# RomanJuranek/librectify

Measured on AMD Instinct MI355X. Metric: Mpix/s end-to-end (detect+VP) on 4K frames, batch call of 64 frames, 5 in flight, higher is better.
Workload: dtype f32

## Files before the change

### librectify_amd/csrc/batch.hip

```cpp
#include "host.h"

#include <cstdio>
#include <cstdlib>
#include <cstring>
#include <string>

namespace lramd {


class LaneSet {
public:
    LaneSet() = default;
    LaneSet(const LaneSet&) = delete;
    LaneSet& operator=(const LaneSet&) = delete;
    int setup(lr_context* caller, int S, bool host_frames, bool keep_workspace) {
        c = caller;
        c->workers.reserve((size_t)std::max(0, S - 1));
        while ((int)c->workers.size() < S - 1) {
            lr_context* wc = nullptr;
            if (ctx_create(c->device, &wc)) return 1;
            c->workers.push_back(wc);
        }
        lanes.reserve((size_t)S);
        lanes.push_back(c);
        for (int i = 0; i < S - 1; ++i) lanes.push_back(c->workers[i]);
        for (lr_context* l : lanes) {
            l->opt = c->opt;
            l->flood_log_min = S == 1 ? 0 : 32;
            l->flood_log_walk = S == 1 ? 0 : 24;
            l->flood_logbig_off = S > 1;
            l->flood_jit_sleep_us = S == 1 ? 0 : 20;
            static const bool sleep_env = std::getenv("LIBRECTIFY_LANES_SLEEP") != nullptr;
            l->sleep_in_wait = sleep_env && host_frames;
            l->keep_workspace = keep_workspace;
        }
        return 0;
    }
    ~LaneSet() {
        if (!c) return;
        for (lr_context* l : lanes) {
            l->sleep_in_wait = false;
            l->keep_workspace = false;
        }
        c->flood_logbig_off = false;
        c->flood_log_min = c->flood_log_walk = 0;
        c->flood_jit_sleep_us = 0;
    }
    int size() const { return (int)lanes.size(); }
    lr_context* operator[](int i) const { return lanes[(size_t)i]; }

private:
    lr_context* c = nullptr;
    std::vector<lr_context*> lanes;
};

struct BatchOut {
    LineSegment* out;
    int capacity;
    int* n_lines;
    const RectificationConfig* cfg;
    ImageTransform* transforms;
    void write(int b, const std::vector<LineSegment>& res, int w, int h) const {
        const int n = (int)res.size();
        if (n_lines) n_lines[b] = n;
        if (out && capacity > 0 && n > 0) std::memcpy(out + (size_t)b * capacity, res.data(), sizeof(LineSegment) * (size_t)std::min(n, capacity));
        if (transforms) {
            const RectificationConfig def;
            transforms[b] = rectification_transform(res.data(), std::min(n, capacity > 0 ? capacity : n), w, h, cfg ? *cfg : def);
        }
    }
};

template <class Frame>
static int run_lanes(const LaneSet& lanes, int batch, std::atomic<int>& stop, const Frame& frame) {
    const int S = lanes.size();
    std::atomic<int> next_frame{0};
    std::vector<int> rc((size_t)S, 0);
    std::vector<std::string> err((size_t)S);
    auto work = [&](int si) {
        bool failed = false;
        if (si > 0 && hipSetDevice(lanes[0]->device) != hipSuccess) {
            set_error("hipSetDevice failed");
            failed = true;
        }
        while (!failed && !stop.load(std::memory_order_relaxed)) {
            const int b = next_frame.fetch_add(1, std::memory_order_relaxed);
            if (b >= batch) break;
            failed = frame(lanes[si], si, b) != 0;
        }
        if (failed) {
            rc[(size_t)si] = 1;
            err[(size_t)si] = get_error();
            stop.store(1);
        }
    };
    {
        JoinedThreads workers;
        for (int si = 1; si < S; ++si) workers.th.emplace_back(work, si);
        work(0);
    }
    for (int si = 0; si < S; ++si)
        if (rc[(size_t)si]) {
            set_error(err[(size_t)si]);
            return 1;
        }
    return 0;
}

int ctx_find_groups_batch_device(lr_context* c, const void* d_images, int format, size_t image_stride, int batch, int w, int h,
                                 int stride, float min_length, bool refine, LineSegment* out, int capacity, int* n_lines,
                                 const RectificationConfig* cfg, ImageTransform* transforms) {
    if (batch <= 0) return 0;
    const size_t bpp = (size_t)pix_bytes(format);
    if (bpp == 0) {
        set_error("unknown pixel format of the frames");
        return 1;
    }
    LaneSet lanes;
    if (lanes.setup(c, std::max(1, std::min(c->opt.batch_streams, batch)), false, false)) return 1;
    const BatchOut results{out, capacity, n_lines, cfg, transforms};
    std::atomic<int> stop{0};
    return run_lanes(lanes, batch, stop, [&](lr_context* l, int, int b) {
        std::vector<LineSegment> res;
        if (ctx_find_groups_device(l, static_cast<const uint8_t*>(d_images) + (size_t)b * image_stride * bpp, format, w, h, stride, min_length,
                                   refine, res))
            return 1;
        results.write(b, res, w, h);
        return 0;
    });
}

int ctx_find_groups_frames_device(lr_context* c, const lr_frame* frames, int format, bool tagged, int batch, float min_length,
                                  bool refine, LineSegment* out, int capacity, int* n_lines, const RectificationConfig* cfg,
                                  ImageTransform* transforms) {
    auto bad = [](int b, const char* what) {
        set_error("lr_find_line_segment_groups_batch_device: frame " + std::to_string(b) + " of the table: " + what);
        return 1;
    };
    if (pix_bytes(format) == 0) {
        set_error("unknown pixel format of the frames");
        return 1;
    }
    if (frames == nullptr) {
        set_error("lr_find_line_segment_groups_batch_device: no frame table");
        return 1;
    }
    size_t max_pix = 0;
    int max_tiles = 0;
    for (int b = 0; b < batch; ++b) {
        const lr_frame& f = frames[b];
        if (f.data == nullptr) return bad(b, "null data");
        if (f.width < 1 || f.height < 1) return bad(b, "size below 1");
        if (f.stride < f.width) return bad(b, "stride smaller than the width");
        if (format == LR_PIX_F32 && (reinterpret_cast<uintptr_t>(f.data) & 3u)) return bad(b, "f32 address not 4-byte aligned");
        if (f.width < 5 || f.height < 5) {
            if (!tagged) return bad(b, "image smaller than the 5x5 filter");
            continue;
        }
        max_pix = std::max(max_pix, (size_t)f.width * (size_t)f.height);
        max_tiles = std::max(max_tiles, filter_geometry(f.width, f.height).n_tiles);
    }
    LaneSet lanes;
    if (lanes.setup(c, std::max(1, std::min(c->opt.batch_streams, batch)), false, true)) return 1;
    LR_HIP(hipSetDevice(c->device));
    for (int si = 0; si < lanes.size() && max_pix; ++si)
        if (ctx_reserve_workspace(lanes[si], max_pix, max_tiles)) return 1;
    const BatchOut results{out, capacity, n_lines, cfg, transforms};
    std::atomic<int> stop{0};
    return run_lanes(lanes, batch, stop, [&](lr_context* l, int, int b) {
        const lr_frame& f = frames[b];
        std::vector<LineSegment> res;
        if (f.width >= 5 && f.height >= 5 &&
            ctx_find_groups_device(l, f.data, format, f.width, f.height, f.stride, f.min_length < 0.f ? min_length : f.min_length, refine, res))
            return 1;
        results.write(b, res, f.width, f.height);
        return 0;
    });
}

int ctx_find_groups_batch_host(lr_context* c, const void* const* frames, int format, int batch, int w, int h, int stride,
                               float min_length, bool refine, int num_threads, LineSegment* out, int capacity,
                               int* n_lines, const RectificationConfig* cfg, ImageTransform* transforms) {
    if (batch <= 0) return 0;
    const int bpp = pix_bytes(format);
    if (bpp == 0) {
        set_error("unknown pixel format of the frames");
        return 1;
    }
    const int S = std::max(1, std::min(c->opt.batch_streams, batch));
    BatchUploader up(c, frames, batch, w, h, stride, bpp, S, num_threads);
    if (up.check()) return 1;
    LaneSet lanes;
    if (lanes.setup(c, S, true, false) || up.start()) return 1;
    const BatchOut results{out, capacity, n_lines, cfg, transforms};
    const int lanes_rc = run_lanes(lanes, batch, up.stop, [&](lr_context* l, int si, int b) {
        const void* img = nullptr;
        int slot = -1;
        if (up.ready(b, l->stream, &img, &slot)) return 1;
        if (img == nullptr) return 0;
        std::vector<LineSegment> res;
        const double t_f0 = now_ms();
        if (ctx_find_groups_device(l, img, format, w, h, w, min_length, refine, res)) return 1;
        up.release(slot, b, l, si, t_f0);
        results.write(b, res, w, h);
        return 0;
    });
    const std::string& up_err = up.end();
    if (lanes_rc) return 1;
    if (!up_err.empty()) {
        set_error(up_err);
        return 1;
    }
    return 0;
}

int ctx_find_groups_batch_host_multi(lr_context* c, const int* devices, int n_devices, const void* const* frames, int format, int batch,
                                     int w, int h, int stride, float min_length, bool refine, int num_threads,
                                     LineSegment* out, int capacity, int* n_lines, const RectificationConfig* cfg,
                                     ImageTransform* transforms) {
    if (batch <= 0) return 0;
    if (n_devices <= 0 || devices == nullptr) {
        set_error("multi-device batch: empty device list");
        return 1;
    }
    int ndev = 0;
    if (hipGetDeviceCount(&ndev) != hipSuccess) ndev = 0;
    for (int i = 0; i < n_devices; ++i)
        if (devices[i] < 0 || devices[i] >= ndev) {
            set_error("multi-device batch: device index out of range");
            return 1;
        }
    if ((int)c->peers.size() > n_devices) {
        for (size_t i = (size_t)n_devices; i < c->peers.size(); ++i) ctx_destroy(c->peers[i]);
        c->peers.resize((size_t)n_devices);
    }
    c->peers.resize((size_t)n_devices, nullptr);
    for (int i = 0; i < n_devices; ++i) {
        if (c->peers[(size_t)i] && c->peers[(size_t)i]->device != devices[i]) {
            ctx_destroy(c->peers[(size_t)i]);
            c->peers[(size_t)i] = nullptr;
        }
        if (!c->peers[(size_t)i] && ctx_create(devices[i], &c->peers[(size_t)i])) {
            (void)hipSetDevice(c->device);
            return 1;
        }
        c->peers[(size_t)i]->opt = c->opt;
    }
    const int per = (batch + n_devices - 1) / n_devices;
    bool blocks_apart = true;
    if (const size_t fbpp = (size_t)pix_bytes(format)) {
        const size_t span = (size_t)(h - 1) * (size_t)(stride < 0 ? -stride : stride) * fbpp + (size_t)w * fbpp;
        for (int i = 0; i < batch && blocks_apart && w > 0 && h > 0; ++i)
            for (int j = (i / per + 1) * per; j < batch && blocks_apart; ++j) {
                if (!frames[i] || !frames[j]) continue;
                const uintptr_t a = reinterpret_cast<uintptr_t>(frames[i]) - (stride < 0 ? (size_t)(h - 1) * (size_t)(-stride) * fbpp : 0);
                const uintptr_t b = reinterpret_cast<uintptr_t>(frames[j]) - (stride < 0 ? (size_t)(h - 1) * (size_t)(-stride) * fbpp : 0);
                blocks_apart = a + span <= b || b + span <= a;
            }
    }
    for (lr_context* p : c->peers) p->batch_no_register = !blocks_apart;
    std::vector<int> rc((size_t)n_devices, 0);
    std::vector<std::string> err((size_t)n_devices);
    auto run = [&](int i) {
        const int b0 = std::min(batch, i * per), b1 = std::min(batch, b0 + per);
        if (b1 <= b0) return;
        lr_context* p = c->peers[(size_t)i];
        if (hipSetDevice(p->device) != hipSuccess) {
            rc[(size_t)i] = 1;
            err[(size_t)i] = "hipSetDevice failed";
            return;
        }
        const int nt = num_threads > 1 ? std::max(2, num_threads / std::min(n_devices, (batch + per - 1) / per)) : num_threads;
        if (ctx_find_groups_batch_host(p, frames + b0, format, b1 - b0, w, h, stride, min_length, refine, nt,
                                       out ? out + (size_t)b0 * capacity : nullptr, capacity, n_lines ? n_lines + b0 : nullptr, cfg,
                                       transforms ? transforms + b0 : nullptr)) {
            rc[(size_t)i] = 1;
            err[(size_t)i] = get_error();
        }
    };
    std::vector<std::thread> th;
    for (int i = 1; i < n_devices; ++i) th.emplace_back(run, i);
    run(0);
    for (auto& t : th) t.join();
    (void)hipSetDevice(c->device);
    for (int i = 0; i < n_devices; ++i)
        if (rc[(size_t)i]) {
            set_error("device list entry " + std::to_string(i) + " (device " + std::to_string(devices[i]) + "): " + err[(size_t)i]);
// ... 7 lines not shown
```

### librectify_amd/csrc/common.h

```cpp
#pragma once
#include <hip/hip_runtime.h>

#include <cstdint>
#include <string>

#include "../../include/librectify_amd.h"

namespace lramd {

constexpr float kEps = 1e-6f;
constexpr int kMaxModels = 4;
constexpr int kMaxPeelModels = 5;
constexpr float kInlierDeg = 2.0f;
constexpr float kGarbageDeg = 4.0f;
constexpr int kRansacMaxIter = 10000;
constexpr int kEdgeKernelSize = 2;
constexpr float kEdgeKernelSigma = 1.0f;
constexpr int kSeedDist = 2;
constexpr float kSeedRatio = 0.95f;
constexpr float kTraceTolerance = 0.25f;
constexpr float kLineMaxErr = 2.0f;
constexpr float kLineMinLength = 5.f;
constexpr int kComponentMinSize = 5;
constexpr int kBins = 8;
constexpr int kOverlayStrokeNum = 9, kOverlayStrokeDen = 4;
constexpr int kOverlayDiscR2 = 25;
constexpr int kOverlayColours = 12;
constexpr uint32_t kOverlayPalette[kOverlayColours] = {0x0000FFu, 0x00FF00u, 0xFF0000u, 0xFFFF00u, 0xFF00FFu, 0x00FFFFu,
                                                       0x000080u, 0x008000u, 0x800000u, 0x808000u, 0x800080u, 0x008080u};
constexpr uint32_t kOverlayUngrouped = 0xFFFFFFu;
constexpr int kOverlayMaxCoord = 1 << 24;

struct FilterConsts {
    float d[5];
    float g[5];
    float st[kBins];
    float ct[kBins];
};

struct BinTrig {
    float st[kBins];
    float ct[kBins];
};

constexpr uint32_t kLabelFree = 0xFFFFFFFFu;

__host__ __device__ inline float directional(float dx, float dy, float s, float c) {
    return fabsf(fmaf(dx, s, dy * c));
}

__host__ __device__ inline uint64_t splitmix64(uint64_t x) {
    x += 0x9E3779B97F4A7C15ull;
    x = (x ^ (x >> 30)) * 0xBF58476D1CE4E5B9ull;
    x = (x ^ (x >> 27)) * 0x94D049BB133111EBull;
    return x ^ (x >> 31);
}
__host__ __device__ inline void sample_pair(uint64_t seed, uint32_t round, uint32_t iter, uint32_t n, uint32_t& a,
                                            uint32_t& b) {
    const uint64_t z = splitmix64(seed ^ splitmix64(((uint64_t)round << 32) | iter));
    const uint32_t u1 = (uint32_t)z, u2 = (uint32_t)(z >> 32);
    const uint32_t i = (uint32_t)(((uint64_t)u1 * n) >> 32);
    uint32_t j = (uint32_t)(((uint64_t)u2 * (n - 1)) >> 32);
    if (j >= i) ++j;
    a = i < j ? i : j;
    b = i < j ? j : i;
}

void set_error(const std::string& msg);

#define LR_HIP(expr)                                                                                     \
    do {                                                                                                 \
        hipError_t _e = (expr);                                                                          \
        if (_e != hipSuccess) {                                                                          \
            (void)hipGetLastError();        \
            ::lramd::set_error(std::string(#expr) + ": " + hipGetErrorString(_e) + " (" + __FILE__ + ":" + \
                               std::to_string(__LINE__) + ")");                                          \
            return 1;                                                                                    \
        }                                                                                                \
    } while (0)

inline int pix_bytes(int format) { return format == LR_PIX_U8 ? 1 : format == LR_PIX_U8X3 ? 3 : format == LR_PIX_F32 ? 4 : 0; }
int launch_filter(const void* img, int format, int w, int h, int stride, const FilterConsts& fc, float* dx, float* dy,
                  uint8_t* dmask, uint64_t* cand, uint32_t* cand_count, uint32_t* tile_max, hipStream_t s);
int filter_band_rows();
int filter_band_last_row(int by);
int launch_filter_rows(const void* img, int format, int w, int h, int stride, const FilterConsts& fc, float* dx, float* dy,
                       uint8_t* dmask, uint64_t* cand, uint32_t* cand_count, uint32_t* tile_max, int by_begin, int by_end,
                       hipStream_t s);
struct FilterGeom {
    int n_tiles;
    int cand_cap;
};
FilterGeom filter_geometry(int w, int h);

size_t seeds_temp_bytes(int n_tiles, size_t max_seeds);
int launch_seed_select(const uint64_t* cand, const uint32_t* cand_count, const uint32_t* tile_max, int n_tiles,
                       int cand_cap, float seed_keep_ratio, float* maxmag, uint32_t* tile_pass, uint32_t* tile_off, uint64_t* keys,
                       uint32_t key_cap, uint32_t* n_seeds, uint32_t frame_tag, hipStream_t s);
int launch_seed_order(uint64_t* keys, uint64_t* keys_alt, const uint32_t* n_seeds, uint32_t cap, const float* dx, const float* dy,
                      BinTrig trig, float trace_tolerance, int32_t* seed_idx, int32_t* seed_bin, float* seed_thr, uint4* seed_rec, hipStream_t s);

int launch_label_init(uint32_t* label, size_t n, hipStream_t s);
int launch_flood_ordered(const float* dx, const float* dy, const uint8_t* dmask, int w, int h, const int32_t* seed_idx,
                         const int32_t* seed_bin, const float* seed_thr, const uint32_t* d_n_seeds, uint32_t seed_cap,
                         BinTrig trig, uint32_t* label, int32_t* seed_size, int32_t* queue, hipStream_t s);

constexpr size_t kFloodHandWords = 1024;
struct FloodBuffers {
    uint32_t* blocked = nullptr;
    uint32_t* count = nullptr;
    uint32_t* flags = nullptr;
    uint8_t* state = nullptr;
    uint8_t* tier = nullptr;
    uint32_t* blk = nullptr;
    uint32_t* act_a = nullptr;
    uint32_t* act_b = nullptr;
    uint32_t* ctrl = nullptr;
    uint8_t* dirty = nullptr;
    uint32_t* big_list = nullptr;
    uint32_t* handover = nullptr;
    bool rewalk_logs = false;
    uint32_t* rewalk_list = nullptr;
    int log_min_tiles = 0, log_walk_tiles = 0;
    bool giant_hold = false;
    bool giant_step = true;
    void* giant_mask = nullptr;
    uint32_t* giant_parent = nullptr;
    bool log_sweep = false;
    bool rewalk_big = false;
    uint32_t log_seeds = 0, log_cap = 0;
    uint32_t* log_off = nullptr;
    uint32_t* log_len = nullptr;
    uint32_t* log_buf = nullptr;
    void* slab_ring = nullptr;
    void* slab_hash = nullptr;
    uint32_t n_slabs = 0, slab_ring_cap = 0, slab_hash_cap = 0;
    int win_first_shift = 0, win_growth = 2;
    int win_hold_pct = 80;
    bool partial_commits = true;
    bool second_tier = true;
    bool second_tier_from_start = true;
    bool hold_from_start = false;
    bool staged_from_start = false;
    int blind_rounds = 10;
    uint32_t* host_progress = nullptr;
    bool calm_hint = false;
    uint32_t* host_ctrl = nullptr;
    int jit_first = 0;
    int jit_sleep_us = 0;
// ... 116 lines not shown
```

### librectify_amd/csrc/context.h

```cpp
#pragma once
#include <atomic>
#include <functional>
#include <memory>
#include <mutex>
#include <vector>

#include "buffers.h"
#include "common.h"
#include "vp_host.h"

namespace lramd {
struct StagingCrew;

struct Settings {
    uint64_t ransac_seed = 0;
    int ransac_iters = kRansacMaxIter;
    int estimator = 0;
    int prosac_T_N = -1;
    int cht_d = 128;
    int batch_streams = 5;
    int flood_mode = 1;
    bool flood_giant_step = true;
    bool flood_jit = true;
    bool flood_partial = true;
// ... 29 lines not shown
    HugeSort huge;
};

struct FloodStore {
    DeviceBuffer<uint32_t> blocked, count, flags, blk, act_a, act_b, ctrl, big_list, handover, rewalk_list, log_off, log_len, log_buf;
    DeviceBuffer<uint8_t> state, tier, dirty;
    DeviceBuffer<uint64_t> giant_mask;
    DeviceBuffer<uint4> slab_ring, slab_hash;
    FloodBuffers fb;
    size_t cap_seeds = 0;
};

struct FrameSlots {
    DeviceBuffer<float> slot[2];
    PinnedBuffer<float> stage[2];
    DeviceBuffer<float> packed;
    DeviceBuffer<float> luma;
};

struct UploadRing {
    std::vector<DeviceBuffer<float>> img;
    std::vector<PinnedBuffer<float>> stage;
    size_t cap_pix = 0, stage_cap_pix = 0;
    void drop() {
        for (auto& b : img) b.reset();
        for (auto& b : stage) b.reset();
        cap_pix = stage_cap_pix = 0;
    }
};

struct PrepareSpans {
    MirroredBuffer<unsigned char> spans;
    int key[4] = {0, 0, 0, 0};
    float w_in[2] = {0.f, 0.f};
    MirroredBuffer<unsigned char> ragged;
};

struct OverlayStore {
    MirroredBuffer<unsigned char> block;
};

struct JpegStore {
    MirroredBuffer<unsigned char> block;
    DeviceBuffer<int16_t> coef;
    DeviceBuffer<uint32_t> len;
    DeviceBuffer<unsigned long long> place;
    DeviceBuffer<unsigned long long> counts;
};

struct JpegDecodeStore {
    MirroredBuffer<unsigned char> block;
    DeviceBuffer<int16_t> coef;
    DeviceBuffer<unsigned long long> state;
    DeviceBuffer<uint32_t> part;
};
}

struct lr_context {
    lr_context();
    ~lr_context();
    int device = 0;
    lramd::Stream stream, copy_stream;
    lramd::Settings opt;

    int w = 0, h = 0;
    lramd::Workspace ws;
    lramd::FloodStore flood;
    lramd::FrameSlots frames;
    lramd::UploadRing ring;
    lramd::PrepareSpans prep;
    lramd::Event ev_prep_spans;
    lramd::Event ev_prep_ragged;
    lramd::OverlayStore overlay;
    lramd::Event ev_overlay;
    lramd::JpegStore jpeg;

    lramd::Event ev_up[2];
    lramd::Event ev_wait;
    std::vector<lramd::Event> band_ev;
    std::vector<lramd::Event> ring_ev;
    std::unique_ptr<lramd::StagingCrew> crew;
    int crew_helpers = 0;
    bool sleep_in_wait = false;
    uint32_t fit_tag = 0;
    bool batch_no_register = false;
    int register_slow_calls = 0;
    uint32_t select_tag = 0;
    lramd::DeviceBuffer<float> maxmag;
    lramd::DeviceBuffer<uint32_t> d_counts;
    uint32_t seed_cap = 0;
    uint32_t seed_cap_once = 0;
    int frame_laps = 0;
    lramd::FloodProgress flood_prog;
    bool keep_workspace = false;
    int small_frames = 0;
    size_t cap_glines = 0;
    lramd::DeviceBuffer<float> d_tables;
    lramd::DeviceBuffer<uint32_t> d_orig;
    lramd::DeviceBuffer<float> d_inl;
    lramd::DeviceBuffer<LineSegment> d_flines;
    lramd::DeviceBuffer<uint32_t> d_gctl;
    lramd::DeviceBuffer<float> d_gnorm;
    lramd::DeviceBuffer<float> d_models;
    lramd::PinnedBuffer<uint8_t> h_res;
    size_t res_lines_cap = 0;
    lramd::DeviceBuffer<float> d_refine_table;
    lramd::DeviceBuffer<uint2> d_refine_edges;
    lramd::DeviceBuffer<unsigned long long> d_cht_acc;
    lramd::MirroredBuffer<uint32_t> cht_idx;
    lramd::MirroredBuffer<uint32_t> cht_peak;
    lramd::MirroredBuffer<double> warp_m;
    lramd::Event ev_warp_m;
    lramd::MirroredBuffer<float> model;
    lramd::DeviceBuffer<unsigned long long> d_best_slots;
    lramd::MirroredBuffer<int32_t> pairs;
    lramd::DeviceBuffer<float> d_peak;
    lramd::MirroredBuffer<float> weights;
    lramd::MirroredBuffer<uint32_t> samples;
    lramd::MirroredBuffer<uint32_t> hcounts;
    lramd::MirroredBuffer<uint32_t> rec;
    lramd::MirroredBuffer<uint8_t> recflags;
    lramd::Event prosac_ev[2];
    std::vector<int> prosac_imin;
    std::vector<lr_context*> workers;
    std::vector<lr_context*> peers;
    lramd::PinnedBuffer<uint32_t> h_counts;
    lramd::PinnedBuffer<float> h_best;

    lramd::FilterConsts fconsts;
    lramd::BinTrig trig;
    float seed_keep_ratio = 0.f;

    uint32_t n_seeds = 0, n_comp = 0, n_px = 0;
    int flood_rounds = 0;
    int flood_rounds_hint = 10;
    int flood_rounds_last = 0;
    int flood_jit_sleep_us = 0;
    bool flood_logbig_off = false;
    int flood_log_min = 0, flood_log_walk = 0;
    bool flood_logbig_hint = true;
    bool flood_big_hint = true;
    bool flood_hold_hint = false;
    int flood_staged_streak = 0;
    bool flood_staged_hint = false;
    bool flood_calm_hint = false;
    uint32_t flood_tiers[16] = {0, 0, 0, 0, 0, 0, 0, 0, 0, 0, 0, 0, 0, 0, 0, 0};
    lramd::Event ev[16];
    float stage_ms[LR_T_COUNT] = {};
    double host_ms[3] = {0, 0, 0};
    bool stage_valid[4] = {false, false, false, false};
    bool dmask_consumed = false;
    lramd::JpegDecodeStore jpeg_decode;
};

namespace lramd {
constexpr size_t kResHeaderBytes = 256;
int ctx_create(int device, lr_context** out);
void ctx_destroy(lr_context* c);
const std::string& get_error();
int ctx_ensure_image_capacity(lr_context* c, int w, int h);
int ctx_reserve_workspace(lr_context* c, size_t npix, int ntiles);
int ctx_trim(lr_context* c, bool frames_too);
int ctx_ensure_ransac_capacity(lr_context* c, size_t n_lines);
int ctx_stage_filter(lr_context* c, const float* d_image, int w, int h, int stride);
int ctx_stage_seeds(lr_context* c);
int ctx_stage_flood(lr_context* c);
// ... 74 lines not shown
```

### librectify_amd/csrc/frame.hip

```cpp
#include "host.h"

#include <cstdio>
#include <cstdlib>
#include <cstring>

namespace lramd {


namespace {

uint32_t round_up(uint32_t v, uint32_t m) { return (v + m - 1) / m * m; }

uint32_t initial_seed_cap(size_t npix) {
    return (uint32_t)std::min<size_t>(npix, std::max<size_t>(round_up((uint32_t)(npix / 32), 1024), 4096));
}

uint32_t line_cap_for(const lr_context* c) {
    return (uint32_t)std::min<size_t>(c->seed_cap, c->ws.cap_pix / 6 + 16);
}


PencilTable table_of(lr_context* c, int which) {
    const size_t cl = c->cap_glines;
    float* b = c->d_tables + (size_t)which * 8 * cl;
// ... 307 lines not shown
    c->stage_valid[1] = true;
    return 0;
}

int ctx_stage_flood(lr_context* c) {
    if (!c->stage_valid[1]) {
        set_error(c->dmask_consumed ? "lr_stage_flood: the previous flood consumed the filter output; run lr_stage_filter and lr_stage_seeds again"
                                    : "lr_stage_flood: run lr_stage_seeds first");
        return 1;
    }
    TimingOn t(c);
    if (enqueue_flood(c)) return 1;
    LR_HIP(hipStreamSynchronize(c->stream));
    bool extra;
    if (finish_flood(c, &extra)) return 1;
    c->stage_valid[2] = true;
    return 0;
}

int ctx_stage_fit(lr_context* c, std::vector<LineSegment>& out) {
    if (!c->stage_valid[2]) {
        set_error("lr_stage_fit: run lr_stage_flood first");
        return 1;
    }
    out.clear();
    TimingOn t(c);
    if (enqueue_fit(c)) return 1;
    LR_HIP(hipMemcpyAsync(c->h_counts, c->d_counts, 8 * sizeof(uint32_t), hipMemcpyDeviceToHost, c->stream));
    LR_HIP(hipStreamSynchronize(c->stream));
    c->n_comp = c->h_counts[kCntComp];
    c->n_px = c->h_counts[kCntPx];
    if (c->n_comp > 0) {
        out.resize(c->n_comp);
        LR_HIP(hipMemcpyAsync(out.data(), c->ws.d_lines, (size_t)c->n_comp * sizeof(LineSegment), hipMemcpyDeviceToHost,
                              c->stream));
        LR_HIP(hipStreamSynchronize(c->stream));
    }
    c->stage_valid[3] = true;
    record_stage_times(c, false);
    return 0;
}

int ctx_detect(lr_context* c, const float* d_image, int w, int h, int stride, std::vector<LineSegment>& raw) {
    if (ctx_stage_filter(c, d_image, w, h, stride)) return 1;
    if (ctx_stage_seeds(c)) return 1;
    if (ctx_stage_flood(c)) return 1;
    return ctx_stage_fit(c, raw);
}

int run_frame(lr_context* c, const void* d_image, int format, int w, int h, int stride, float min_length, bool refine,
              std::vector<LineSegment>& out, bool filter_enqueued) {
    out.clear();
    const double t_begin = now_ms();
    const bool fused = !refine && c->opt.estimator == 0;
    const int n_iter = c->opt.ransac_iters;
    auto groups_after_fit = [&]() -> int {
        const uint32_t lc = line_cap_for(c);
        if (ensure_group_capacity(c, lc)) return 1;
        if (ensure_result_block(c, std::max<size_t>(c->res_lines_cap, 4096))) return 1;
        if (c->opt.timing_on) LR_HIP(hipEventRecord(c->ev[5], c->stream));
        const PencilTable all = table_of(c, 0), round0 = table_of(c, 1);
        if (launch_filter_lines(c->ws.d_lines, c->d_counts + kCntComp, lc, min_length, c->d_flines, c->d_gctl, c->d_gnorm, &all, &round0,
                                c->stream))
            return 1;
        static_assert(kMaxModels >= 1 && kGcWords == 8 && kResHeaderBytes == 256, "the last peeling round carries the result block (peel_kernel)");
        if (enqueue_groups(c, lc, kMaxModels, kInlierDeg, kGarbageDeg, n_iter, c->opt.ransac_seed, true, true)) return 1;
        if (c->opt.timing_on) LR_HIP(hipEventRecord(c->ev[6], c->stream));
        return 0;
    };
    auto after_fit = [&]() -> int {
        if (fused) return groups_after_fit();
        LR_HIP(hipMemcpyAsync(c->h_counts, c->d_counts, 8 * sizeof(uint32_t), hipMemcpyDeviceToHost, c->stream));
        return 0;
    };
    c->frame_laps = 0;
    for (int attempt = 0;; ++attempt) {
        c->frame_laps += 1;
        if (!(filter_enqueued && attempt == 0) && enqueue_filter(c, d_image, format, w, h, stride)) return 1;
        if (enqueue_seeds(c)) return 1;
        if (enqueue_flood(c)) return 1;
        if (enqueue_fit(c)) return 1;
        if (after_fit()) return 1;
        const double t_enq = now_ms();
        const double t_pre = now_ms();
        if (c->sleep_in_wait) {
            LR_HIP(hipEventRecord(c->ev_wait, c->stream));
            LR_HIP(hipEventSynchronize(c->ev_wait));
        } else {
            LR_HIP(hipStreamSynchronize(c->stream));
        }
        c->host_ms[0] = t_enq - t_begin;
        c->host_ms[1] = t_pre - t_enq;
        c->host_ms[2] = now_ms() - t_pre;
        const uint32_t* cnt = fused ? reinterpret_cast<const uint32_t*>(c->h_res.get()) : c->h_counts.get();
        c->n_seeds = cnt[kCntSeeds];
        if (c->n_seeds <= c->seed_cap) break;
        if (attempt > 0) {
            set_error("seed count exceeds the sort capacity twice");
            return 1;
        }
        adapt_seed_cap(c, c->n_seeds);
    }
    bool extra = false;
    if (finish_flood(c, &extra)) return 1;
    if (extra) {
        c->frame_laps += 1;
        if (enqueue_fit(c)) return 1;
        if (after_fit()) return 1;
        LR_HIP(hipStreamSynchronize(c->stream));
    }
    const uint32_t* cnt = fused ? reinterpret_cast<const uint32_t*>(c->h_res.get()) : c->h_counts.get();
    c->n_comp = cnt[kCntComp];
    c->n_px = cnt[kCntPx];
    adapt_seed_cap(c, c->n_seeds);
    c->stage_valid[0] = c->stage_valid[1] = false;
    c->stage_valid[2] = c->stage_valid[3] = true;
    if (fused) {
        const uint32_t* gctl = reinterpret_cast<const uint32_t*>(c->h_res + 32);
        const size_t n = gctl[kGcLines];
        out.resize(n);
        const size_t have = std::min<size_t>(n, c->res_lines_cap);
        if (have) std::memcpy(out.data(), c->h_res + kResHeaderBytes, have * sizeof(LineSegment));
        if (n > have) {
            LR_HIP(hipMemcpyAsync(out.data() + have, c->d_flines + have, (n - have) * sizeof(LineSegment),
                                  hipMemcpyDeviceToHost, c->stream));
            LR_HIP(hipStreamSynchronize(c->stream));
            if (ensure_result_block(c, round_up((uint32_t)(n + n / 2), 1024))) return 1;
        }
        record_stage_times(c, true);
#ifdef LR_PEEL_TIMING
        {
            const float* tm = reinterpret_cast<const float*>(c->h_res + 64) + 16;
            for (int r = 0; r < 4; ++r)
                std::fprintf(stderr, "peel round %d: best %.1f us, inliers %.1f, sums %.1f, jacobi %.1f, verdict %.1f\n", r,
                             tm[r * 5], tm[r * 5 + 1], tm[r * 5 + 2], tm[r * 5 + 3], tm[r * 5 + 4]);
        }
#endif
        return 0;
    }
    std::vector<LineSegment> raw(c->n_comp);
    if (c->n_comp) {
        LR_HIP(hipMemcpyAsync(raw.data(), c->ws.d_lines, (size_t)c->n_comp * sizeof(LineSegment), hipMemcpyDeviceToHost,
                              c->stream));
        LR_HIP(hipStreamSynchronize(c->stream));
    }
    record_stage_times(c, false);
    if (raw.size() < 2) return 0;
    if (refine && ctx_refine(c, raw)) return 1;
    std::vector<LineSegment> filtered = filter_lines(raw, min_length);
    if (filtered.empty()) return 0;
    if (c->opt.timing_on) LR_HIP(hipEventRecord(c->ev[5], c->stream));
    if (c->opt.estimator == 1) {
        if (ctx_estimate_line_pencils_prosac(c, filtered, kMaxModels, kInlierDeg, kGarbageDeg, c->opt.prosac_T_N,
                                             c->opt.ransac_seed))
            return 1;
    } else if (c->opt.estimator == 2) {
        if (ctx_estimate_line_pencils_direct(c, filtered, kMaxModels, kInlierDeg, kGarbageDeg)) return 1;
    } else if (c->opt.estimator == 3) {
        if (ctx_estimate_line_pencils_cht(c, filtered, kMaxModels, kInlierDeg, kGarbageDeg, c->opt.cht_d, nullptr)) return 1;
    } else if (ctx_estimate_line_pencils(c, filtered, kMaxModels, kInlierDeg, kGarbageDeg, n_iter, c->opt.ransac_seed)) {
        return 1;
    }
    if (c->opt.timing_on) LR_HIP(hipEventRecord(c->ev[6], c->stream));
    LR_HIP(hipStreamSynchronize(c->stream));
    record_stage_times(c, true);
    out.swap(filtered);
// ... 145 lines not shown
```

### librectify_amd/csrc/kernels_filter.hip

```cpp
#include <algorithm>
#include <cstdlib>
#include <cstring>

#include "common.h"

namespace lramd {
namespace {

struct FilterTaps {
    float d1, d2, g1, g2;
    float st[kBins];
    float ct[kBins];
};

#ifndef LR_BAND_ROWS
#define LR_BAND_ROWS 30
#endif
constexpr int kBandRows = LR_BAND_ROWS;
constexpr int kBandSteps = kBandRows + 8;

__device__ __forceinline__ float from_lower(float v) {
    const int i = __float_as_int(v);
    return __int_as_float(__builtin_amdgcn_mov_dpp(i, 0x138 , 0xF, 0xF, true));
}
// ... 66 lines not shown
template <int kFormat, int K10>
__device__ __forceinline__ void lane_step(Roll1<typename Px<kFormat>::Q>& R, const int t, const void* __restrict__ img, const int w, const int h,
                                          const int stride, const FilterTaps& fc, float* __restrict__ dx_out,
                                          float* __restrict__ dy_out, uint8_t* __restrict__ dmask_out,
                                          uint64_t* __restrict__ cand_band, uint32_t& ncand, float& lmax, const int y0,
                                          const int x, const int xcl, const int lane, const bool useful,
                                          const BufRsrc r_img, const BufRsrc r_dx, const BufRsrc r_dy,
                                          const BufRsrc r_dm) {
    constexpr int K = K10 % 5;
    if (t >= kBandSteps) return;
    const float cur = Px<kFormat>::value(R.q[K10]);
    {
        const int yy = min(max(y0 - 4 + t + 9, 0), h - 1);
        R.q[(K10 + 9) % 10] = Px<kFormat>::fetch(r_img, (unsigned)xcl, (unsigned)yy * (unsigned)stride);
    }
    const float l1 = from_lower(cur), r1 = from_upper(cur);
    const float l2 = from_lower(l1), r2 = from_upper(r1);
    R.hx[K] = fmaf(r2 - l2, fc.d2, (r1 - l1) * fc.d1);
    R.hs[K] = fmaf(r2 + l2, fc.g2, fmaf(r1 + l1, fc.g1, cur));
    if (t < 4) return;

    const int yc = y0 - 6 + t;
    const float ax = fmaf(R.hx[K] + R.hx[(K + 1) % 5], fc.g2,
                          fmaf(R.hx[(K + 4) % 5] + R.hx[(K + 2) % 5], fc.g1, R.hx[(K + 3) % 5]));
    const float ay = fmaf(R.hs[K] - R.hs[(K + 1) % 5], fc.d2, (R.hs[(K + 4) % 5] - R.hs[(K + 2) % 5]) * fc.d1);
    const bool ok = (yc >= 2) && (yc < h - 2) && (x >= 2) && (x < w - 2);
    const float vx = ok ? ax : 0.f;
    const float vy = ok ? ay : 0.f;
    R.mag[K] = sqrtf(vx * vx + vy * vy);
    float g[kBins];
#pragma unroll
    for (int b = 0; b < kBins; ++b) g[b] = directional(vx, vy, fc.st[b], fc.ct[b]);

    const float gm = fmaxf(fmaxf(fmaxf(g[0], g[1]), fmaxf(g[2], g[3])), fmaxf(fmaxf(g[4], g[5]), fmaxf(g[6], g[7])));
    uint32_t bit = 1u << 7;
#pragma unroll
    for (int b = kBins - 2; b >= 0; --b) bit = (g[b] == gm) ? (1u << b) : bit;
    R.bits[K] = bit;
    const bool in_img = useful && x < w;
    if (t >= 6 && t < 6 + kBandRows && yc < h) {
        if (in_img) {
            const unsigned row = (unsigned)yc * (unsigned)w * 4u;
            __builtin_amdgcn_raw_buffer_store_b32(__builtin_bit_cast(int, vx), r_dx, (unsigned)x * 4u, row, 0);
            __builtin_amdgcn_raw_buffer_store_b32(__builtin_bit_cast(int, vy), r_dy, (unsigned)x * 4u, row, 0);
        }
    }
    if (t < 8) return;

    const int yo = yc - 2;
    if (yo >= h) return;
    const float cm = fmaxf(fmaxf(fmaxf(R.mag[0], R.mag[1]), fmaxf(R.mag[2], R.mag[3])), R.mag[4]);
    const float cl1 = from_lower(cm), cr1 = from_upper(cm);
    const float cl2 = from_lower(cl1), cr2 = from_upper(cr1);
    const float mx = fmaxf(fmaxf(fmaxf(cl2, cl1), fmaxf(cm, cr1)), cr2);
    const float c = R.mag[(K + 3) % 5];
    const uint32_t cb = R.bits[(K + 3) % 5];
    const uint32_t v = R.bits[(K + 2) % 5] | cb | R.bits[(K + 4) % 5];
    uint32_t dm = from_lower(v) | v | from_upper(v);
    if (yo == 0 || yo == h - 1 || x == 0 || x == w - 1) dm = 0;
    if (in_img) {
        lmax = fmaxf(lmax, c);
        __builtin_amdgcn_raw_buffer_store_b8((unsigned char)dm, r_dm, (unsigned)x, (unsigned)yo * (unsigned)w, 0);
    }
    const bool peak = in_img && (yo >= 2) && (yo < h - 2) && (x >= 2) && (x < w - 2) && (c > 0.f) && (c == mx);
    const uint64_t m = __ballot(peak);
    if (m) {
        if (peak) {
            const uint32_t idx = (uint32_t)yo * (uint32_t)w + (uint32_t)x;
            const uint32_t pb = (uint32_t)__ffs((int)cb) - 1u;
            cand_band[ncand + (uint32_t)__popcll(m & ((1ull << lane) - 1ull))] =
                ((uint64_t)__float_as_uint(c) << 32) | (uint64_t)((idx << 3) | pb);
        }
        ncand += (uint32_t)__popcll(m);
    }
}

template <int kFormat>
__global__ __launch_bounds__(256) void filter_lanes_kernel(const void* __restrict__ img, int w, int h, int stride,
                                                           FilterTaps fc, float* __restrict__ dx_out,
                                                           float* __restrict__ dy_out, uint8_t* __restrict__ dmask_out,
                                                           uint64_t* __restrict__ cand, uint32_t* __restrict__ cand_count,
                                                           uint32_t* __restrict__ tile_max, int bands_x, int band_begin,
                                                           int band_end) {
    const int lane = threadIdx.x & 63;
#ifndef LR_NO_XCD_ORDER
    const int chunk = (int)gridDim.x / 8;
    const int wg = (int)(blockIdx.x & 7u) * chunk + (int)(blockIdx.x >> 3);
#else
    const int wg = (int)blockIdx.x;
#endif
    const int band = __builtin_amdgcn_readfirstlane(band_begin + wg * 4 + (int)(threadIdx.x >> 6));
    if (band >= band_end) return;
    const int by = band / bands_x, bx = band - by * bands_x;
    const int y0 = by * kBandRows;
    const int x = bx * kLaneCols - 4 + lane;
    const int xcl = min(max(x, 0), w - 1);
    const bool useful = lane >= 4 && lane <= 59;
    using P = Px<kFormat>;
    Roll1<typename P::Q> R;
#pragma unroll
    for (int i = 0; i < 5; ++i) {
        R.hx[i] = 0.f;
        R.hs[i] = 0.f;
        R.mag[i] = 0.f;
        R.bits[i] = 1u;
    }
#pragma unroll
    for (int i = 0; i < 10; ++i) R.q[i] = (i < 9) ? P::first(img, stride, h, y0 - 4 + i, xcl) : typename P::Q(0);
    uint64_t* cand_band = cand + (size_t)band * (kLaneCols * kBandRows);
    uint32_t ncand = 0;
    float lmax = 0.f;
    const uint32_t npx = (uint32_t)w * (uint32_t)h;
    const BufRsrc r_img = make_rsrc(img, ((uint32_t)(h - 1) * (uint32_t)stride + (uint32_t)w) * P::kBytes);
    const BufRsrc r_dx = make_rsrc(dx_out, npx * 4u), r_dy = make_rsrc(dy_out, npx * 4u), r_dm = make_rsrc(dmask_out, npx);
#define LR_STEP(k) lane_step<kFormat, k>(R, t0 + k, img, w, h, stride, fc, dx_out, dy_out, dmask_out, cand_band, ncand, lmax, y0, x, xcl, lane, useful, r_img, r_dx, r_dy, r_dm)
#pragma unroll
    for (int t0 = 0; t0 < (kBandSteps + 9) / 10 * 10; t0 += 10) {
        LR_STEP(0); LR_STEP(1); LR_STEP(2); LR_STEP(3); LR_STEP(4);
        LR_STEP(5); LR_STEP(6); LR_STEP(7); LR_STEP(8); LR_STEP(9);
    }
#undef LR_STEP
#pragma unroll
    for (int off = 32; off >= 1; off >>= 1) lmax = fmaxf(lmax, __shfl_xor(lmax, off));
    if (lane == 0) {
        tile_max[band] = __float_as_uint(lmax);
        cand_count[band] = ncand;
    }
}

}

FilterGeom filter_geometry(int w, int h) {
    FilterGeom g;
    g.n_tiles = ((w + kLaneCols - 1) / kLaneCols) * ((h + kBandRows - 1) / kBandRows);
    g.cand_cap = kLaneCols * kBandRows;
    return g;
}

static int filter_taps(const FilterConsts& fc, FilterTaps& ft) {
    if (!(fc.d[2] == 0.f && fc.g[2] == 1.f && fc.d[1] == -fc.d[3] && fc.d[0] == -fc.d[4] && fc.g[1] == fc.g[3] &&
          fc.g[0] == fc.g[4])) {
        set_error("launch_filter: derivative factors are not (anti)symmetric on this host");
        return 1;
    }
    ft.d1 = fc.d[3];
    ft.d2 = fc.d[4];
    ft.g1 = fc.g[3];
    ft.g2 = fc.g[4];
    for (int b = 0; b < kBins; ++b) {
        ft.st[b] = fc.st[b];
        ft.ct[b] = fc.ct[b];
    }
    return 0;
}

int filter_band_rows() { return kBandRows; }
int filter_band_last_row(int by) { return kBandRows * by - 4 + kBandSteps - 1; }

int launch_filter_rows(const void* img, int format, int w, int h, int stride, const FilterConsts& fc, float* dx, float* dy,
                       uint8_t* dmask, uint64_t* cand, uint32_t* cand_count, uint32_t* tile_max, int by_begin, int by_end,
                       hipStream_t s) {
    if (w < 1 || h < 1 || stride < w) {
        set_error("launch_filter: bad geometry");
        return 1;
    }
    if (format != LR_PIX_F32 && format != LR_PIX_U8) {
// ... 33 lines not shown
```

### librectify_amd/csrc/kernels_fit.hip

```cpp
#include <algorithm>
#include <cstring>

#include <atomic>

#include "common.h"

namespace lramd {
namespace {

constexpr uint32_t kNoComp = 0xFFFFFFFFu;

constexpr uint32_t kSortLds = 1024;
constexpr uint32_t kSortLdsBig = 16384;
constexpr uint32_t kHugeShift = 14;
constexpr uint32_t kHugeFlag = 0x80000000u;
constexpr int kOffPer = 8;
constexpr uint32_t kOffChunk = 256 * kOffPer;

__device__ __forceinline__ void chunk_counts(const int32_t* __restrict__ seed_size, uint32_t n_seeds, int min_size,
                                             uint32_t k0, int (&sz)[kOffPer], uint32_t& c, uint32_t& p) {
    c = p = 0;
#pragma unroll
    for (int j = 0; j < kOffPer; ++j) {
        sz[j] = (k0 + j < n_seeds) ? seed_size[k0 + j] : 0;
        if (sz[j] > min_size) {
            c += 1u;
            p += (uint32_t)sz[j];
        }
    }
}

__global__ __launch_bounds__(256) void component_offsets_kernel(const int32_t* __restrict__ seed_size,
                                                                const uint32_t* __restrict__ n_ptr, uint32_t cap,
                                                                int min_size, unsigned long long* __restrict__ status, uint32_t tag,
                                                                uint32_t* __restrict__ comp_rank,
                                                                uint32_t* __restrict__ comp_seed,
                                                                uint32_t* __restrict__ comp_off,
                                                                uint32_t* __restrict__ totals,
                                                                uint32_t* __restrict__ large_list,
                                                                uint32_t large_cap, uint32_t* __restrict__ n_large,
                                                                uint32_t* __restrict__ cursor, uint32_t* __restrict__ huge_list,
                                                                uint32_t huge_max) {
    __shared__ uint32_t s_c[4], s_p[4], s_cc[4], s_cp[4];
    const uint32_t n_seeds = min(*n_ptr, cap);
    const int tid = threadIdx.x, lane = tid & 63, wv = tid >> 6;
    const uint32_t k0 = blockIdx.x * kOffChunk + (uint32_t)tid * kOffPer;
    int sz[kOffPer];
    uint32_t c, p;
    chunk_counts(seed_size, n_seeds, min_size, k0, sz, c, p);
    uint32_t ic = c, ip = p;
#pragma unroll
    for (int off = 1; off < 64; off <<= 1) {
        const uint32_t tc = (uint32_t)__shfl_up((int)ic, off);
        const uint32_t tp = (uint32_t)__shfl_up((int)ip, off);
        if (lane >= off) {
            ic += tc;
            ip += tp;
        }
    }
    if (lane == 63) {
        s_c[wv] = ic;
        s_p[wv] = ip;
    }
    __syncthreads();
    if (tid == 0) {
        const unsigned long long t = (unsigned long long)tag << 32;
        const unsigned long long wc = t | (unsigned long long)(s_c[0] + s_c[1] + s_c[2] + s_c[3]);
        const unsigned long long wp = t | (unsigned long long)(s_p[0] + s_p[1] + s_p[2] + s_p[3]);
        if (blockIdx.x == 0) {
#pragma unroll
            for (int i = 0; i < 4; ++i) __hip_atomic_store(&n_large[i], 0u, __ATOMIC_RELAXED, __HIP_MEMORY_SCOPE_AGENT);
            __hip_atomic_store(&status[0], wc, __ATOMIC_RELEASE, __HIP_MEMORY_SCOPE_AGENT);
            __hip_atomic_store(&status[1], wp, __ATOMIC_RELEASE, __HIP_MEMORY_SCOPE_AGENT);
        } else {
            __hip_atomic_store(&status[2u * blockIdx.x], wc, __ATOMIC_RELAXED, __HIP_MEMORY_SCOPE_AGENT);
            __hip_atomic_store(&status[2u * blockIdx.x + 1u], wp, __ATOMIC_RELAXED, __HIP_MEMORY_SCOPE_AGENT);
        }
    }
    uint32_t cc = 0, cp = 0;
    for (uint32_t i = (uint32_t)tid; i < blockIdx.x; i += 256) {
        unsigned long long wc = 0ull, wp = 0ull;
        for (uint32_t spins = 0; spins < (1u << 22); ++spins) {
            wc = __hip_atomic_load(&status[2u * i], __ATOMIC_RELAXED, __HIP_MEMORY_SCOPE_AGENT);
            wp = __hip_atomic_load(&status[2u * i + 1u], __ATOMIC_RELAXED, __HIP_MEMORY_SCOPE_AGENT);
            if ((uint32_t)(wc >> 32) == tag && (uint32_t)(wp >> 32) == tag) break;
            __builtin_amdgcn_s_sleep(2);
        }
        cc += (uint32_t)wc;
        cp += (uint32_t)wp;
    }
#pragma unroll
    for (int off = 32; off >= 1; off >>= 1) {
        cc += (uint32_t)__shfl_xor((int)cc, off);
        cp += (uint32_t)__shfl_xor((int)cp, off);
    }
    if (lane == 0) {
        s_cc[wv] = cc;
        s_cp[wv] = cp;
    }
    __syncthreads();
    uint32_t rank = s_cc[0] + s_cc[1] + s_cc[2] + s_cc[3] + ic - c;
    uint32_t off_px = s_cp[0] + s_cp[1] + s_cp[2] + s_cp[3] + ip - p;
    for (int i = 0; i < wv; ++i) {
        rank += s_c[i];
        off_px += s_p[i];
    }
#pragma unroll
    for (int j = 0; j < kOffPer; ++j) {
        const uint32_t k = k0 + j;
        if (k < n_seeds) {
            const bool keep = sz[j] > min_size;
            comp_rank[k] = keep ? rank : kNoComp;
            if (keep) {
                comp_seed[rank] = k;
                comp_off[rank] = off_px;
                if (sz[j] > (int)kSortLds) large_list[large_cap - 1u - atomicAdd(n_large + 1, 1u)] = rank;
                else if (sz[j] > 64) large_list[atomicAdd(n_large, 1u)] = rank;
                uint32_t cur = 0u;
                if (sz[j] > (int)kSortLdsBig && huge_max != 0u) {
                    const uint32_t hi = atomicAdd(n_large + 2, 1u);
                    if (hi < huge_max) {
                        cur = hi | kHugeFlag;
                        huge_list[hi] = rank;
                    }
                }
                cursor[rank] = cur;
                rank += 1u;
                off_px += (uint32_t)sz[j];
            }
        }
    }
    if (blockIdx.x == gridDim.x - 1 && tid == 255) {
        totals[0] = rank;
        totals[1] = off_px;
        comp_off[rank] = off_px;
    }
}

__global__ __launch_bounds__(256) void component_scatter_kernel(const uint32_t* __restrict__ label, size_t npix,
                                                                const uint32_t* __restrict__ comp_rank,
                                                                const uint32_t* __restrict__ comp_off,
                                                                uint32_t* __restrict__ cursor,
                                                                uint32_t* __restrict__ px, uint32_t* __restrict__ huge_tab,
                                                                uint32_t nb) {
    const int lane = threadIdx.x & 63;
    const size_t step = (size_t)gridDim.x * 256;
    const size_t n_pad = (npix + 255) / 256 * 256;
    constexpr int kU = 4;
    for (size_t i0 = (size_t)blockIdx.x * 256 + threadIdx.x; i0 < n_pad; i0 += step * kU) {
        uint32_t l[kU], r[kU];
#pragma unroll
        for (int u = 0; u < kU; ++u) {
            const size_t i = i0 + step * (size_t)u;
            l[u] = i < npix ? label[i] : kLabelFree;
        }
#pragma unroll
        for (int u = 0; u < kU; ++u) r[u] = l[u] != kLabelFree ? comp_rank[l[u]] : kNoComp;
#pragma unroll
        for (int u = 0; u < kU; ++u) {
            const size_t i = i0 + step * (size_t)u;
            if (i >= n_pad) break;
            uint64_t todo = __ballot(r[u] != kNoComp);
            while (todo != 0ull) {
                const int leader = __builtin_ctzll(todo);
                const uint32_t rl = (uint32_t)__builtin_amdgcn_readlane((int)r[u], leader);
                const uint64_t same = __ballot(r[u] == rl) & todo;
                uint32_t base = 0;
                if (lane == leader) {
                    const uint32_t o0 = comp_off[rl], o1 = comp_off[rl + 1u];
                    uint32_t hi = 0u;
                    if (o1 - o0 > kSortLdsBig) hi = cursor[rl];
                    if (hi & kHugeFlag) base = atomicAdd(&huge_tab[(size_t)(hi & ~kHugeFlag) * nb + (uint32_t)(i >> kHugeShift)], (uint32_t)__popcll(same));
                    else base = o0 + atomicAdd(&cursor[rl], (uint32_t)__popcll(same));
                }
                base = (uint32_t)__builtin_amdgcn_readlane((int)base, leader);
                if ((same >> lane) & 1ull) px[base + (uint32_t)__popcll(same & ((1ull << lane) - 1ull))] = (uint32_t)i;
                todo &= ~same;
            }
        }
    }
}

__device__ inline float wave_tree(float v) {
#pragma unroll
    for (int off = 32; off >= 1; off >>= 1) v = v + __shfl_xor(v, off);
    return v;
}

__device__ inline void major_axis_2x2(float a_, float b_, float c_, float& d_r, float& d_c) {
    const double a = a_, b = b_, c = c_;
    const double hd = (a - c) * 0.5;
    const double rad = sqrt(hd * hd + b * b);
    const double lmax = (a + c) * 0.5 + rad;
    double vr, vc;
    if (a >= c) {
        vr = lmax - c;
        vc = b;
    } else {
        vr = b;
        vc = lmax - a;
    }
    const double nn = sqrt(vr * vr + vc * vc);
    if (nn > 0.0) {
        vr = vr / nn;
        vc = vc / nn;
    } else {
        vr = 1.0;
        vc = 0.0;
    }
    float fr = (float)vr, fc = (float)vc;
    if (fr < fc || (fr == fc && fr < 0.0f)) {
        fr = -fr;
        fc = -fc;
    }
    d_r = fr;
    d_c = fc;
}

template <int kThreads, class Keys>
__device__ __forceinline__ void bitonic_sort(Keys& key, uint32_t P) {
    for (uint32_t k = 2; k <= P; k <<= 1)
        for (uint32_t j = k >> 1; j > 0; j >>= 1) {
            for (uint32_t t = threadIdx.x; t < P / 2; t += kThreads) {
                const uint32_t i = 2 * t - (t & (j - 1));
                const uint32_t a = key[i], b = key[i + j];
                const bool up = (i & k) == 0;
                if ((a > b) == up) {
                    key[i] = b;
                    key[i + j] = a;
                }
            }
            __syncthreads();
        }
}

__global__ __launch_bounds__(256) void component_sort_large_kernel(const uint32_t* __restrict__ px_in,
                                                                   uint32_t* __restrict__ px_out,
                                                                   const uint32_t* __restrict__ comp_off,
                                                                   const uint32_t* __restrict__ large_list,
                                                                   const uint32_t* __restrict__ n_large) {
    __shared__ uint32_t s_key[kSortLds];
    const uint32_t n_list = n_large[0];
    for (uint32_t li = blockIdx.x; li < n_list; li += gridDim.x) {
        const uint32_t comp = large_list[li];
        const uint32_t off = comp_off[comp];
        const uint32_t n = comp_off[comp + 1] - off;
        uint32_t P = 128;
        while (P < n) P <<= 1;
        for (uint32_t i = threadIdx.x; i < P; i += 256) s_key[i] = i < n ? px_in[off + i] : 0xFFFFFFFFu;
        __syncthreads();
        bitonic_sort<256>(s_key, P);
        for (uint32_t i = threadIdx.x; i < n; i += 256) px_out[off + i] = s_key[i];
        __syncthreads();
    }
}

template <bool kGlobal>
__global__ __launch_bounds__(1024) void component_sort_big_kernel(const uint32_t* __restrict__ px_in,
                                                                  uint32_t* __restrict__ px_out,
                                                                  const uint32_t* __restrict__ comp_off,
                                                                  const uint32_t* __restrict__ large_list,
                                                                  uint32_t large_cap,
                                                                  const uint32_t* __restrict__ n_large,
                                                                  uint32_t* __restrict__ scratch,
                                                                  const uint32_t* __restrict__ cursor) {
    __shared__ uint32_t s_key[kGlobal ? 1 : kSortLdsBig];
    const uint32_t n_list = n_large[1];
    for (uint32_t li = blockIdx.x; li < n_list; li += gridDim.x) {
        const uint32_t comp = large_list[large_cap - 1u - li];
        const uint32_t off = comp_off[comp];
        const uint32_t n = comp_off[comp + 1] - off;
        if ((n > kSortLdsBig) != kGlobal) continue;
        if (kGlobal && cursor != nullptr && (cursor[comp] & kHugeFlag)) continue;
        uint32_t P = 2048;
        while (P < n) P <<= 1;
        if (!kGlobal) {
            for (uint32_t i = threadIdx.x; i < P; i += 1024) s_key[i] = i < n ? px_in[off + i] : 0xFFFFFFFFu;
            __syncthreads();
            bitonic_sort<1024>(s_key, P);
            for (uint32_t i = threadIdx.x; i < n; i += 1024) px_out[off + i] = s_key[i];
            __syncthreads();
        } else {
            for (uint32_t i = threadIdx.x; i < P; i += 1024) scratch[i] = i < n ? px_in[off + i] : 0xFFFFFFFFu;
            __syncthreads();
            bitonic_sort<1024>(scratch, P);
            for (uint32_t i = threadIdx.x; i < n; i += 1024) px_out[off + i] = scratch[i];
            __syncthreads();
        }
    }
}

__global__ __launch_bounds__(256) void huge_count_kernel(const uint32_t* __restrict__ label, size_t npix,
                                                         const uint32_t* __restrict__ comp_rank,
                                                         const uint32_t* __restrict__ comp_off,
                                                         const uint32_t* __restrict__ cursor, uint32_t* __restrict__ huge_tab,
                                                         uint32_t nb, const uint32_t* __restrict__ huge_list, uint32_t huge_max,
                                                         uint4* __restrict__ jobs, uint32_t* __restrict__ n_large) {
    const uint32_t n_huge = min(n_large[2], huge_max);
    if (n_huge == 0u) return;
    const int lane = threadIdx.x & 63;
    const size_t step = (size_t)gridDim.x * 256;
    const size_t n_pad = (npix + 255) / 256 * 256;
    for (size_t i = (size_t)blockIdx.x * 256 + threadIdx.x; i < n_pad; i += step) {
        const uint32_t l = i < npix ? label[i] : kLabelFree;
        const uint32_t r = l != kLabelFree ? comp_rank[l] : kNoComp;
        uint32_t hi = 0u;
        if (r != kNoComp && comp_off[r + 1u] - comp_off[r] > kSortLdsBig) hi = cursor[r];
        uint64_t todo = __ballot((hi & kHugeFlag) != 0u);
        while (todo != 0ull) {
            const int leader = __builtin_ctzll(todo);
            const uint32_t hl = (uint32_t)__builtin_amdgcn_readlane((int)hi, leader);
            const uint64_t same = __ballot(hi == hl) & todo;
            if (lane == leader) atomicAdd(&huge_tab[(size_t)(hl & ~kHugeFlag) * nb + (uint32_t)(i >> kHugeShift)], (uint32_t)__popcll(same));
            todo &= ~same;
        }
    }
    __shared__ uint32_t s_last;
    __syncthreads();
    if (threadIdx.x == 0) {
        __threadfence();
        s_last = atomicAdd(n_large + 6, 1u) == gridDim.x - 1u ? 1u : 0u;
    }
    __syncthreads();
    if (s_last == 0u) return;
    __threadfence();
    if (threadIdx.x == 0) n_large[6] = 0u;
    for (uint32_t h = threadIdx.x >> 6; h < n_huge; h += 4u) {
        const uint32_t rank = huge_list[h];
        uint32_t run = comp_off[rank];
        for (uint32_t b0 = 0; b0 < nb; b0 += 64u) {
            const uint32_t b = b0 + (uint32_t)lane;
            uint32_t* e = &huge_tab[(size_t)h * nb + b];
            const uint32_t cnt = b < nb ? __hip_atomic_load(e, __ATOMIC_RELAXED, __HIP_MEMORY_SCOPE_AGENT) : 0u;
            uint32_t inc = cnt;
#pragma unroll
            for (int off = 1; off < 64; off <<= 1) {
                const uint32_t t = (uint32_t)__shfl_up((int)inc, off);
                if (lane >= off) inc += t;
            }
            const uint32_t start = run + inc - cnt;
            if (cnt != 0u) {
                *e = start;
                jobs[atomicAdd(n_large + 3, 1u)] = make_uint4(start, cnt, h * nb + b, 0u);
            }
            run += (uint32_t)__shfl((int)inc, 63);
        }
    }
}
// ... 65 lines not shown
                const float wn = wq[u] / S;
                ar = ar + wn * r;
                ac = ac + wn * cc;
            }
        }
    }
    const float a_r = wave_tree(ar), a_c = wave_tree(ac);

    float crr = 0.f, crc = 0.f, ccc = 0.f;
    for (uint32_t i0 = lane; i0 < n; i0 += 64u * kU) {
        uint32_t p[kU];
        float wq[kU];
#pragma unroll
        for (int u = 0; u < kU; ++u) {
            const uint32_t i = i0 + 64u * (uint32_t)u;
            p[u] = i < n ? px[off + i] : 0u;
            wq[u] = i < n ? scratch_w[off + i] : 0.f;
        }
#pragma unroll
        for (int u = 0; u < kU; ++u) {
            const uint32_t i = i0 + 64u * (uint32_t)u;
            if (i < n) {
                const float cr = (float)(p[u] / uw) - a_r, cc = (float)(p[u] % uw) - a_c;
                const float wn = wq[u] / S;
                const float t = cr * wn, u2 = cc * wn;
                crr = crr + t * cr;
                crc = crc + t * cc;
                ccc = ccc + u2 * cc;
            }
        }
    }
    const float cov_rr = wave_tree(crr), cov_rc = wave_tree(crc), cov_cc = wave_tree(ccc);

    float d_r, d_c;
    major_axis_2x2(cov_rr, cov_rc, cov_cc, d_r, d_c);
    const float n_r = -d_c, n_c = d_r;

    float t0 = INFINITY, t1 = -INFINITY, es = 0.f;
    for (uint32_t i0 = lane; i0 < n; i0 += 64u * kU) {
        uint32_t p[kU];
#pragma unroll
        for (int u = 0; u < kU; ++u) {
            const uint32_t i = i0 + 64u * (uint32_t)u;
            p[u] = i < n ? px[off + i] : 0u;
        }
#pragma unroll
        for (int u = 0; u < kU; ++u) {
            const uint32_t i = i0 + 64u * (uint32_t)u;
            if (i < n) {
                const float cr = (float)(p[u] / uw) - a_r, cc = (float)(p[u] % uw) - a_c;
                const float t = cr * d_r + cc * d_c;
                t0 = fminf(t0, t);
                t1 = fmaxf(t1, t);
                es = es + fabsf(cr * n_r + cc * n_c);
            }
        }
    }
#pragma unroll
    for (int o = 32; o >= 1; o >>= 1) {
        t0 = fminf(t0, __shfl_xor(t0, o));
        t1 = fmaxf(t1, __shfl_xor(t1, o));
    }
    const float esum = wave_tree(es);
    if (lane == 0) {
        LineSegment l;
        l.x1 = a_c + d_c * t0;
        l.y1 = a_r + d_r * t0;
        l.x2 = a_c + d_c * t1;
        l.y2 = a_r + d_r * t1;
        l.weight = S / (float)n;
        l.err = esum / (float)n;
        l.group_id = -1;
        out[comp] = l;
    }
}

__global__ __launch_bounds__(256) void fit_kernel(const uint32_t* __restrict__ px, const uint32_t* __restrict__ px_unsorted,
                                                  const uint32_t* __restrict__ comp_off,
                                                  const uint32_t* __restrict__ comp_seed, const uint32_t* __restrict__ n_comp_ptr,
                                                  const int32_t* __restrict__ seed_bin, const float* __restrict__ dx,
                                                  const float* __restrict__ dy, int w, BinTrig trig,
                                                  float* __restrict__ scratch_w, LineSegment* __restrict__ out,
                                                  const uint32_t* __restrict__ huge_cursor) {
    const int lane = threadIdx.x & 63;
    const uint32_t comp = blockIdx.x * 4 + (threadIdx.x >> 6);
    if (comp >= *n_comp_ptr) return;
    const uint32_t off = comp_off[comp];
    const uint32_t n = comp_off[comp + 1] - off;
    const int b = seed_bin[comp_seed[comp]];
    const float s = trig.st[b], c = trig.ct[b];
    const uint32_t uw = (uint32_t)w;

    if (n <= 64u) {
        const bool has = (uint32_t)lane < n;
        const uint32_t key = has ? px_unsorted[off + lane] : 0xFFFFFFFFu;
        uint32_t rank = 0;
#pragma unroll
        for (int j = 0; j < 64; ++j) rank += ((uint32_t)__builtin_amdgcn_readlane((int)key, j) < key) ? 1u : 0u;
        const uint32_t p_sorted = (uint32_t)__builtin_amdgcn_ds_permute((int)(min(rank, 63u) << 2), (int)key);
        const uint32_t p = has ? p_sorted : 0u;
        float wv = 0.f;
        if (has) wv = directional(dx[p], dy[p], s, c);
        float acc = 0.f;
        if (has) acc = acc + wv;
        const float S = wave_tree(acc);
        const float r = (float)(p / uw), cq = (float)(p % uw);
        const float wn = wv / S;
        float ar = 0.f, ac = 0.f;
        if (has) {
            ar = ar + wn * r;
            ac = ac + wn * cq;
        }
        const float a_r = wave_tree(ar), a_c = wave_tree(ac);
        const float cr = r - a_r, cc = cq - a_c;
        float crr = 0.f, crc = 0.f, ccc = 0.f;
        if (has) {
            const float t = cr * wn, u = cc * wn;
            crr = crr + t * cr;
            crc = crc + t * cc;
            ccc = ccc + u * cc;
        }
        const float cov_rr = wave_tree(crr), cov_rc = wave_tree(crc), cov_cc = wave_tree(ccc);
        float d_r, d_c;
        major_axis_2x2(cov_rr, cov_rc, cov_cc, d_r, d_c);
        const float n_r = -d_c, n_c = d_r;
        float t0 = INFINITY, t1 = -INFINITY, es = 0.f;
        if (has) {
            const float t = cr * d_r + cc * d_c;
            t0 = fminf(t0, t);
            t1 = fmaxf(t1, t);
            es = es + fabsf(cr * n_r + cc * n_c);
        }
#pragma unroll
        for (int o = 32; o >= 1; o >>= 1) {
            t0 = fminf(t0, __shfl_xor(t0, o));
            t1 = fmaxf(t1, __shfl_xor(t1, o));
        }
        const float esum = wave_tree(es);
        if (lane == 0) {
            LineSegment l;
            l.x1 = a_c + d_c * t0;
            l.y1 = a_r + d_r * t0;
            l.x2 = a_c + d_c * t1;
            l.y2 = a_r + d_r * t1;
            l.weight = S / (float)n;
            l.err = esum / (float)n;
            l.group_id = -1;
            out[comp] = l;
        }
        return;
    }

    if (huge_cursor != nullptr && n > kSortLdsBig && (huge_cursor[comp] & kHugeFlag) != 0u) return;
    fit_large<8>(px, comp, off, n, s, c, uw, dx, dy, scratch_w, out, lane);
}

__device__ __forceinline__ float huge_chunk_sum(float acc, const float* __restrict__ v, uint32_t cn, int lane) {
    for (uint32_t j0 = (uint32_t)lane; j0 < cn; j0 += 64u * 16u) {
        float t[16];
#pragma unroll
        for (int u = 0; u < 16; ++u) {
            const uint32_t j = j0 + 64u * (uint32_t)u;
            t[u] = j < cn ? v[j] : 0.f;
        }
#pragma unroll
        for (int u = 0; u < 16; ++u)
// ... 283 lines not shown
```

### librectify_amd/csrc/kernels_flood.hip

```cpp
#include <algorithm>
#include <atomic>
#include <chrono>
#include <cstdio>
#include <cstdlib>
#include <cstring>
#include <thread>
#include <sys/prctl.h>
#include <vector>

#include "common.h"

namespace lramd {
namespace {

__device__ inline uint32_t ld_agent(const uint32_t* p) {
    return __hip_atomic_load(p, __ATOMIC_RELAXED, __HIP_MEMORY_SCOPE_AGENT);
}

__global__ __launch_bounds__(256) void label_init_kernel(uint32_t* __restrict__ label, size_t n) {
    size_t i = (size_t)blockIdx.x * 256 + threadIdx.x;
    const size_t step = (size_t)gridDim.x * 256;
    for (; i < n; i += step) label[i] = kLabelFree;
}

// ... 1011 lines not shown
#ifdef LR_WALK_TIMING
    clk.stamped = __builtin_amdgcn_s_memtime();
#endif
    if (rc == 0 && st.ntiles >= A.log_min_tiles && st.ntiles <= A.log_max_len && k < A.log_seeds && uni(A.log_len[k]) == 0u)
        save_log(A, k, L, st.ntiles, lane);
    if (rc != 0) {
        uint32_t slab = 0;
        if (lane == 0) slab = atomicAdd(&A.ctrl[kCtrlSlabs], 1u);
        slab = (uint32_t)__shfl((int)slab, 0);
        if (slab < A.n_slabs) {
            uint32_t gen = 0;
            if (lane == 0) atomicAdd(&A.ctrl[kCtrlSlabTotal], 1u);
            if (lane == 0) gen = atomicAdd(&A.ctrl[kCtrlGen], 1u) + 1u;
            gen = (uint32_t)__shfl((int)gen, 0);
            SlabStore G{A.slab_ring + (size_t)slab * A.slab_ring_cap, A.slab_hash + (size_t)slab * A.slab_hash_cap * 2,
                        A.slab_ring_cap, A.slab_hash_cap, gen};
            for (uint32_t i = st.head; i != st.tail; ++i) {
                uint32_t t;
                uint64_t m;
                L.get(i, t, m);
                G.put(i, t, m);
            }
            for (int i = 0; i < LdsStore::kHashN; ++i) {
                const uint32_t key = L.hk[i];
                if (key) {
                    uint32_t slot;
                    uint64_t v0;
                    (void)G.lookup(key - 1u, slot, v0);
                    G.update(slot, key - 1u, ((uint64_t)L.hv1[i] << 32) | L.hv0[i]);
                }
            }
            rc = walk(A, k, b, thr, sn, cs, G, P, st, lane, K, own);
        }
        if (rc != 0 && lane == 0) {
            A.flags[k] = kFlagIncomplete;
            atomicMin(&A.ctrl[kCtrlBarrier], k);
        }
    }
    if (lane == 0) {
        A.count[k] = st.cnt;
        if (st.blocked) A.blocked[k] = 1u;
        A.flags[k] |= st.steps << 8;
    }
}

template <bool kRest>
__device__ __forceinline__ void explore_body(const FloodArgs& A, const BinTrig& trig, uint32_t* __restrict__ big_list, uint32_t first) {
    __shared__ uint32_t s_ring[3][kRingT];
    __shared__ uint32_t s_hash[3][kHashT];
    __shared__ uint32_t s_pend[2][kPend];
    __shared__ uint8_t s_ord[kHashT];
#ifdef LR_LDS_PAD
    __shared__ uint32_t s_pad[LR_LDS_PAD / 4];
    asm volatile("" ::"v"(&s_pad[threadIdx.x]) : "memory");
#endif
    const int lane = threadIdx.x & 63;
#ifdef LR_WALK_TIMING
    WalkClock clk{__builtin_amdgcn_s_memtime(), 0, 0, 0};
    const auto clock_out = [&]() {
        const uint64_t now = __builtin_amdgcn_s_memtime();
        unsigned long long* t = g_prologue_timing[blockIdx.x & 63u];
        if (lane == 0) {
            if (clk.first != 0 && clk.stamped != 0) {
                atomicAdd(&t[0], 1ull);
                atomicAdd(&t[1], (unsigned long long)(clk.first - clk.entry));
                atomicAdd(&t[2], (unsigned long long)(clk.walked - clk.first));
                atomicAdd(&t[3], (unsigned long long)(clk.stamped - clk.walked));
            } else {
                atomicAdd(&t[4], 1ull);
                atomicAdd(&t[5], (unsigned long long)(now - clk.entry));
            }
        }
        clk = WalkClock{now, 0, 0, 0};
    };
#endif
    const uint32_t args = walk_args(A);
    const uint32_t* ctrl = A.ctrl;
    uint32_t c_giant = uni(ctrl[kCtrlGiantStep]);
    const uint32_t c_rounds = uni(ctrl[kCtrlRounds]), n_act = uni(ctrl[kCtrlNAct]), window = uni(ctrl[kCtrlWindow]),
                   c_seen = uni(ctrl[kCtrlBigSeen]), c_nbig = uni(ctrl[kCtrlNBig]), lowest = uni(ctrl[kCtrlLowest]),
                   c_staged = uni(ctrl[kCtrlStaged]);
    const uint32_t grid = gridDim.x;
    LR_PIN10(c_giant, c_rounds, n_act, window, c_seen, c_nbig, lowest, c_staged, args, grid);
    if (c_giant != 0u) return;
    const uint32_t* __restrict__ act = (c_rounds & 1u) ? A.act_b : A.act_a;
    const bool staged = c_staged != 0u;
    const uint32_t t1_usual = c_seen != 0u ? kRegionalTiles : 0xFFFFFFFFu;
    const bool tier2_full = A.giant_hold != 0u && A.big_cap != 0u && c_nbig >= A.big_cap;
    LdsStore L{s_ring[0], s_ring[1], s_ring[2], s_hash[0], s_hash[1], s_hash[2], s_ord};
    Pending P{s_pend[0], s_pend[1]};
    if (!kRest) {
        const uint32_t ai = uni(blockIdx.x);
#ifdef LR_WALK_TIMING
        if (ai >= n_act && lane == 0) {
            atomicAdd(&g_prologue_timing[blockIdx.x & 63u][6], 1ull);
            atomicAdd(&g_prologue_timing[blockIdx.x & 63u][7], (unsigned long long)(__builtin_amdgcn_s_memtime() - clk.entry));
        }
#endif
        if (ai >= n_act) return;
        const bool fwd = A.no_rest != 0u && n_act > grid;
        const uint32_t k = uni(act[!fwd ? n_act - 1u - ai : ai]);
        if (k >= window) return;
        const uint32_t t1_tiles = (tier2_full && k != lowest) ? min(t1_usual, kFullTiles) : t1_usual;
        explore_seed(A, trig, k, L, P, big_list, lane, t1_tiles, staged LR_CLOCK_ARG);
#ifdef LR_WALK_TIMING
        clock_out();
#endif
    } else {
        for (uint32_t ai = first + uni(blockIdx.x); ai < n_act; ai += grid) {
            const uint32_t k = uni(act[n_act - 1u - ai]);
            if (k >= window) continue;
            const uint32_t t1_tiles = (tier2_full && k != lowest) ? min(t1_usual, kFullTiles) : t1_usual;
            explore_seed(A, trig, k, L, P, big_list, lane, t1_tiles, staged LR_CLOCK_ARG);
#ifdef LR_WALK_TIMING
            clock_out();
#endif
        }
    }
}
__global__ __launch_bounds__(64) __attribute__((amdgpu_waves_per_eu(4, 8))) void flood_explore_kernel(
    FloodArgs A, BinTrig trig, uint32_t* __restrict__ big_list) {
    explore_body<false>(A, trig, big_list, 0u);
}
__global__ __launch_bounds__(64) __attribute__((amdgpu_waves_per_eu(4, 8))) void flood_explore_rest_kernel(
    FloodArgs A, BinTrig trig, uint32_t* __restrict__ big_list, uint32_t first) {
    explore_body<true>(A, trig, big_list, first);
}

#ifndef LR_TEAM_WAVES
#define LR_TEAM_WAVES 8
#endif
constexpr int kTeamWaves = LR_TEAM_WAVES;
#ifndef LR_TEAM_RING
#define LR_TEAM_RING 1024
#endif
constexpr int kRingTeam = LR_TEAM_RING;
#ifndef LR_TEAM_GRID
#define LR_TEAM_GRID 512
#endif
constexpr uint32_t kTeamGrid = LR_TEAM_GRID;
constexpr uint32_t kVoidTile = 0xFFFFFFFFu;

struct TeamShared {
    uint32_t tail, end, ntiles, blocked, overflow, cnt, steps, pad;
    uint32_t blocker, pad2;
};
__device__ __forceinline__ uint32_t lds_now(const uint32_t* p) {
    return __hip_atomic_load(p, __ATOMIC_RELAXED, __HIP_MEMORY_SCOPE_WORKGROUP);
}

struct TeamStore {
    static constexpr int kHashShift = 32 - __builtin_ctz((unsigned)kHashBig);
    uint32_t* rt;
    uint32_t* rlo;
    uint32_t* rhi;
    uint32_t* hk;
    uint32_t* hv0;
    uint32_t* hv1;
    uint16_t* ord;
    TeamShared* sh;
    __device__ uint32_t hash_limit() const { return kHashBig * 3 / 4; }
    __device__ void get(uint32_t i, uint32_t& tile, uint64_t& m) const {
        const uint32_t j = i & (kRingTeam - 1);
        tile = uni(rt[j]);
        m = uni64(rlo[j], rhi[j]);
    }
// ... 154 lines not shown
        }
    }
}

template <class Store>
__device__ int team_walk(const FloodArgs& A, uint32_t k, int b, float thr, float sn, float cs, Store& S, int lane,
                         int wave, bool own, uint32_t first_level, uint32_t tile_cap, uint32_t* begin_out, uint32_t* steps_out) {
    TeamShared* sh = S.sh;
    const int lr = lane >> 3, lc = lane & 7;
    int rx, ry;
    ring_xy(lane, rx, ry);
    const bool ring_lane = lane < 36;
    const uint64_t adj = ring_adjacency(lane);
    uint64_t nbr = tile_neighbours(lane);
    asm volatile("" : "+v"(nbr));
    const PushLane pc = push_lane(lane);
    const uint32_t bin_bit = 1u << b;
    Forward fw;
    fw.valid = false;
    LaneGeom G;
    G.off = (uint32_t)(lr * A.w + lc);
    G.roff = (uint32_t)(ry * A.w + rx);
    asm volatile("" : "+v"(G.off), "+v"(G.roff));
    uint32_t gb = 0u, ge = first_level, steps = 0u, levels = 0u;
    int rc = 0;
    for (;;) {
        for (uint32_t i = gb + (uint32_t)wave; i < ge; i += kTeamWaves) {
            if ((uni(lds_now(&sh->tail)) - gb) + 8u * kTeamWaves > S.ring_cap() ||
                uni(lds_now(&sh->ntiles)) + kTeamWaves + 1u > min(S.hash_limit(), tile_cap)) {
                if (lane == 0) sh->overflow = 1u;
                break;
            }
            if (uni(lds_now(&sh->overflow)) != 0u) break;
            const TileFetch cur = fetch_tile<0>(A, S, i, lr, lc, rx, ry, ring_lane, fw, G, own);
            ++steps;
            const uint32_t tile = cur.tile;
            uint64_t Am = cur.inside & m_ne(cur.dm & bin_bit, 0u) & m_gt_f(directional(cur.dx, cur.dy, sn, cs), thr);
            uint64_t Rg = cur.rinside & m_ne(cur.rdm & bin_bit, 0u) & m_gt_f(directional(cur.rdx, cur.rdy, sn, cs), thr);
            if (own) {
                Am |= cur.inside & m_eq(cur.lab, k);
                Rg |= cur.rinside & m_eq(cur.rlab, k);
            }
            uint64_t R = cur.entry & Am;
            if (R != 0ull) {
                const uint64_t reach = lane_of(Am) ? nbr : 0ull;
                for (;;) {
                    const uint64_t R1 = m_ne64(R & reach, 0ull);
                    R = m_ne64(R1 & reach, 0ull);
                    if (R == R1) break;
                }
                const uint64_t New = R & ~cur.V;
                if (New != 0ull) {
                    uint64_t was = 0ull;
                    if (lane == 0) was = S.add_walked(cur.slot, New);
                    const uint64_t first_here = New & ~uni64(was);
                    if (first_here != 0ull) {
                        const uint64_t H = Rg & m_ne64(first_here & adj, 0ull);
                        if (H != 0ull) team_push8(S, tile, H, lane, pc);
                    }
                }
            }
            if (lane == 0) S.mark_processed(i);
        }
        __syncthreads();
        if (threadIdx.x == 0) sh->end = sh->tail;
        __syncthreads();
        const uint32_t ne = sh->end;
        if (sh->overflow != 0u || ++levels > kMaxSteps) {
            rc = 1;
            break;
        }
        if (ne == ge) break;
        gb = ge;
        ge = ne;
    }
    *begin_out = gb;
    *steps_out = steps;
    return rc;
}

constexpr size_t kTeamLdsBytes = (size_t)(3 * kRingTeam + 3 * kHashBig + 2 * kPend) * 4 + (size_t)kHashBig * 2 + sizeof(TeamShared);
__global__ __launch_bounds__(64 * kTeamWaves) void flood_explore_team_kernel(FloodArgs A, BinTrig trig,
                                                                             const uint32_t* __restrict__ big_list) {
    extern __shared__ uint32_t s_team[];
    const int lane = threadIdx.x & 63, wave = (int)uni(threadIdx.x >> 6);
    const uint32_t args = walk_args(A);
    uint32_t c_nact = uni(A.ctrl[kCtrlNAct]);
    const uint32_t c_giant = uni(A.ctrl[kCtrlGiantStep]), n_big_raw = uni(A.ctrl[kCtrlNBig]);
    LR_PIN4(c_nact, c_giant, n_big_raw, args);
    if (c_nact == 0u || c_giant != 0u) return;
    const uint32_t n_big = n_big_raw < A.big_cap ? n_big_raw : A.big_cap;
    uint32_t* ring = s_team;
    uint32_t* hash = ring + 3 * kRingTeam;
    uint32_t* pend = hash + 3 * kHashBig;
    uint16_t* ord = reinterpret_cast<uint16_t*>(pend + 2 * kPend);
    TeamShared* sh = reinterpret_cast<TeamShared*>(reinterpret_cast<char*>(ord) + (size_t)kHashBig * 2);
    TeamStore S{ring, ring + kRingTeam, ring + 2 * kRingTeam, hash, hash + kHashBig, hash + 2 * kHashBig, ord, sh};
    for (uint32_t ai = uni(blockIdx.x); ai < n_big; ai += gridDim.x) {
        const uint32_t k = uni(big_list[ai]);
        const uint32_t* hb = A.handover + (size_t)ai * kFloodHandWords;
        const uint4 rec = A.seed_rec[k];
        uint32_t s_u = uni(rec.x);
        const uint32_t b_u = uni(rec.y), thr_u = uni(rec.z), hb_tiles = uni(hb[0]), hb_recs = uni(hb[1]);
        LR_PIN5(s_u, b_u, thr_u, hb_tiles, hb_recs);
        const int s = (int)s_u, b = (int)b_u;
        const float thr = __uint_as_float(thr_u);
        uint32_t seed_label = uni(A.label[s]);
        const uint32_t mask_u = uni(ld8_word(A.dmask, (uint32_t)s));
        const uint32_t dx_u = uni(__float_as_uint(A.dx[s])), dy_u = uni(__float_as_uint(A.dy[s]));
        const uint32_t sn_u = uni(__float_as_uint(trig.st[b])), cs_u = uni(__float_as_uint(trig.ct[b]));
        LR_PIN6(seed_label, mask_u, dx_u, dy_u, sn_u, cs_u);
        const float sn = __uint_as_float(sn_u), cs = __uint_as_float(cs_u);
        const bool own = seed_label == k;
        const bool in_mask = ((byte_of(mask_u, (uint32_t)s) >> b) & 1u) != 0u;
        const bool above = directional(__uint_as_float(dx_u), __uint_as_float(dy_u), sn, cs) > thr;
        const bool accepts = in_mask & above;
        if ((seed_label < kMarkBit) & !own) continue;
        if (!own & !accepts) {
            if (threadIdx.x == 0) A.flags[k] = kFlagSelfFail;
            continue;
        }
        if (A.giant_hold != 0u && k != uni(A.ctrl[kCtrlLowest]) &&
            ((k >= (uni(A.ctrl[kCtrlNSeeds]) >> 2) && giants_many(A.ctrl, A.giant_many)) || giants_all(A.ctrl))) {
            if (threadIdx.x == 0) {
                A.flags[k] = kFlagIncomplete;
                atomicMin(&A.ctrl[kCtrlBarrier], k);
            }
            continue;
        }
        const uint32_t h_recs = min(hb_recs, kHandRecs);
        uint32_t begin = 0u, my_steps = 0u;
        __syncthreads();
        for (int i = (int)threadIdx.x; i < kHashBig; i += 64 * kTeamWaves) {
            S.hk[i] = 0u;
            S.hv0[i] = 0u;
            S.hv1[i] = 0u;
        }
        const uint32_t h_tiles = min(hb_tiles, kHandTiles);
        const uint32_t first_level = h_recs ? h_recs : 1u;
        __syncthreads();
        if (h_recs) {
            for (uint32_t t = threadIdx.x; t < h_tiles; t += 64u * kTeamWaves) {
                const uint32_t key = hb[kHandTable + 3u * t];
                uint32_t hs = (key * 2654435761u) >> TeamStore::kHashShift;
                while (atomicCAS(&S.hk[hs], 0u, key) != 0u) hs = (hs + 1u) & (uint32_t)(kHashBig - 1);
                S.hv0[hs] = hb[kHandTable + 3u * t + 1u];
                S.hv1[hs] = hb[kHandTable + 3u * t + 2u];
                S.ord[t] = (uint16_t)hs;
            }
            for (uint32_t t = threadIdx.x; t < h_recs; t += 64u * kTeamWaves) {
                S.rt[t] = hb[kHandRing + 3u * t];
                S.rlo[t] = hb[kHandRing + 3u * t + 1u];
                S.rhi[t] = hb[kHandRing + 3u * t + 2u];
            }
        }
        if (threadIdx.x == 0) {
            if (!h_recs) {
                const int sr = s / A.w, sc = s - sr * A.w;
                const uint64_t m = 1ull << ((sr & 7) * 8 + (sc & 7));
                S.rt[0] = ((uint32_t)(sr >> 3) << 16) | (uint32_t)(sc >> 3);
                S.rlo[0] = (uint32_t)m;
                S.rhi[0] = (uint32_t)(m >> 32);
            }
            sh->tail = first_level;
            sh->end = first_level;
            sh->ntiles = h_recs ? h_tiles : 0u;
// ... 96 lines not shown
            atomicAdd(&sh->steps, my_steps);
            if (st.blocked) atomicOr(&sh->blocked, 1u);
            if (st.blocker != 0xFFFFFFFFu) atomicMin(&sh->blocker, st.blocker);
        }
        __syncthreads();
        if (wave != 0) continue;
        st.cnt = sh->cnt;
        st.steps = sh->steps;
        st.blocked = sh->blocked != 0u;
        st.blocker = sh->blocker;
        if (rc == 0 && lane == 0 && (A.tier[k] & 4u)) A.tier[k] = (uint8_t)(A.tier[k] & ~4u);
        if (!in_slab && rc == 0 && st.ntiles >= A.log_min_tiles && st.ntiles <= A.log_max_len && k < A.log_seeds &&
            uni(A.log_len[k]) == 0u)
            save_log(A, k, S, st.ntiles, lane);
        if (rc != 0 && lane == 0) {
            A.flags[k] = kFlagIncomplete;
            atomicMin(&A.ctrl[kCtrlBarrier], k);
        }
        if (lane == 0 && A.blk != nullptr) {
            const bool no_log = !(k < A.log_seeds && A.log_min_tiles != 0xFFFFFFFFu && A.log_len[k] != 0u);
            A.blk[k] = (rc == 0 && st.blocked && st.blocker < k && st.steps >= kDeferSteps && k >= (A.ctrl[kCtrlNSeeds] >> 1) && no_log) ? st.blocker : 0xFFFFFFFFu;
        }
        if (lane == 0) {
            A.count[k] = st.cnt;
            if (st.blocked) A.blocked[k] = 1u;
            A.flags[k] |= st.steps << 8;
            if (st.ntiles > kHandTiles) atomicAdd(&A.ctrl[kCtrlBigLong], 1u);
            atomicAdd(&A.ctrl[kCtrlTeamDone], 1u);
        }
    }
}

constexpr int kRwComps = 6;
constexpr uint32_t kRwBatch = 16;
constexpr uint64_t kCol0 = 0x0101010101010101ull, kCol7 = 0x8080808080808080ull;
__device__ __forceinline__ uint64_t dilate8(uint64_t m) {
    const uint64_t hz = m | ((m << 1) & ~kCol0) | ((m >> 1) & ~kCol7);
    return hz | (hz << 8) | (hz >> 8);
}
__device__ __forceinline__ uint32_t rw_find(volatile uint32_t* par, uint32_t x) {
    for (;;) {
        const uint32_t p = par[x];
        if (p == x) return x;
        const uint32_t g = par[p];
        if (g != p) par[x] = g;
        x = g;
    }
}
__device__ __forceinline__ uint32_t rw_order(uint32_t x) { return x * 0x9E3779B1u; }
__device__ __forceinline__ void rw_union(uint32_t* par, uint32_t a, uint32_t b) {
    for (;;) {
        uint32_t ra = rw_find(par, a), rb = rw_find(par, b);
        if (ra == rb) return;
        if (rw_order(ra) < rw_order(rb)) {
            const uint32_t t = ra;
            ra = rb;
            rb = t;
        }
        if (atomicCAS(&par[ra], ra, rb) == ra) return;
    }
}
constexpr int kRewalkTiles = 256;
constexpr uint32_t kRewalkGrid = 2048;
constexpr int kRewalkThreads = 256;
constexpr int kRewalkTilesBig = 2048, kRewalkThreadsBig = 1024;
template <int kTiles>
constexpr size_t rewalk_lds_bytes() {
    return (size_t)kTiles * 3 * 4 + (size_t)2 * kTiles * 4 + (size_t)2 * kTiles * 3 * 4 + (size_t)4 * kTiles * 4 + (size_t)2 * kTiles * 2 +
           (size_t)kTiles * 2 + (size_t)kTiles;
}
#ifdef LR_REWALK_TIMING
__device__ unsigned long long g_rewalk_timing[8];
#define RW_TICK(i)                                            \
    if (threadIdx.x == 0) {                                   \
        const uint64_t t_ = __builtin_amdgcn_s_memtime();     \
        atomicAdd(&g_rewalk_timing[i], (unsigned long long)(t_ - tlast)); \
        tlast = t_;                                           \
    }
#else
#define RW_TICK(i)
#endif
template <int kThreads, int kTiles>
__global__ __launch_bounds__(kThreads) void flood_rewalk_kernel(FloodArgs A, const uint32_t* __restrict__ list, uint32_t min_len) {
    constexpr int kNodes = 2 * kTiles, kHash = 2 * kTiles, kWaves = kThreads / 64, kEdges = 4 * kTiles;
    static_assert(kNodes <= 65536, "node pairs are packed into 32 bits");
    constexpr int kHashShift = 32 - __builtin_ctz((unsigned)kHash);
    extern __shared__ uint32_t s_rw[];
    uint32_t* tid = s_rw;
    uint32_t* mlo = tid + kTiles;
    uint32_t* mhi = mlo + kTiles;
    uint32_t* hkey = mhi + kTiles;
    uint32_t* nlo = hkey + kHash;
    uint32_t* nhi = nlo + kNodes;
    uint32_t* par = nhi + kNodes;
    uint32_t* edge = par + kNodes;
    uint16_t* hidx = reinterpret_cast<uint16_t*>(edge + kEdges);
    uint16_t* tfirst = hidx + kHash;
    uint8_t* tcomp = reinterpret_cast<uint8_t*>(tfirst + kTiles);
    __shared__ uint32_t s_nnodes, s_over, s_blocked, s_cnt, s_seed_node, s_nout, s_nedges;
    const int lane = threadIdx.x & 63, wave = (int)uni(threadIdx.x >> 6);
    const int lr = lane >> 3, lc = lane & 7;
    uint32_t c_nact = uni(A.ctrl[kCtrlNAct]);
    const uint32_t c_giant = uni(A.ctrl[kCtrlGiantStep]), c_nrewalk = uni(A.ctrl[kCtrlNRewalk]), window = uni(A.ctrl[kCtrlWindow]);
    LR_PIN4(c_nact, c_giant, c_nrewalk, window);
    if (c_nact == 0u || c_giant != 0u) return;
    const uint32_t n_list = min(c_nrewalk, kBigCap);
    for (uint32_t ai = uni(blockIdx.x); ai < n_list; ai += gridDim.x) {
        const uint32_t k = uni(list[ai]);
        if (k >= window) continue;
        uint32_t len_w = uni(A.log_len[k]);
        const uint32_t s = uni(A.seed_rec[k].x), log_off = uni(A.log_off[k]);
        LR_PIN3(len_w, s, log_off);
        const uint32_t n = len_w & ~kLogShrunk;
        if (n < min_len || n > (uint32_t)kTiles) continue;
        const uint32_t seed_label = uni(A.label[s]);
        const bool own = seed_label == k;
        if (seed_label < kMarkBit && !own) continue;
        const uint32_t mine = kMarkBit | k;
        uint32_t* rec = A.log_buf + (size_t)log_off * 3u;
        __syncthreads();
#ifdef LR_REWALK_TIMING
        uint64_t tlast = __builtin_amdgcn_s_memtime();
        if (threadIdx.x == 0) {
            atomicAdd(&g_rewalk_timing[0], 1ull);
            atomicAdd(&g_rewalk_timing[1], (unsigned long long)n);
        }
#endif
        for (uint32_t i = threadIdx.x; i < n; i += kThreads) {
            tid[i] = rec[3u * i];
            mlo[i] = rec[3u * i + 1u];
            mhi[i] = rec[3u * i + 2u];
        }
        for (uint32_t i = threadIdx.x; i < (uint32_t)kHash; i += kThreads) hkey[i] = 0u;
        if (threadIdx.x == 0) {
            s_nnodes = 0u;
            s_over = 0u;
            s_blocked = 0u;
            s_cnt = 0u;
            s_seed_node = 0xFFFFFFFFu;
            s_nout = 0u;
            s_nedges = 0u;
        }
        __syncthreads();
        RW_TICK(2)
        for (uint32_t i0 = (uint32_t)wave * kRwBatch; i0 < n; i0 += (uint32_t)kWaves * kRwBatch) {
            uint32_t lab[kRwBatch];
            bool in[kRwBatch];
#pragma unroll
            for (int j = 0; j < (int)kRwBatch; ++j) {
                const uint32_t i = i0 + (uint32_t)j;
                lab[j] = 0u;
                in[j] = false;
                if (i < n) {
                    const uint32_t tile = tid[i];
                    const uint64_t V = ((uint64_t)mhi[i] << 32) | mlo[i];
                    in[j] = (V >> lane) & 1ull;
                    if (in[j]) lab[j] = A.label[(size_t)((tile >> 16) * 8 + lr) * A.w + ((tile & 0xFFFFu) * 8 + lc)];
                }
            }
#pragma unroll
            for (int j = 0; j < (int)kRwBatch; ++j) {
                const uint32_t i = i0 + (uint32_t)j;
                const uint64_t M = __ballot(in[j] && (lab[j] >= kMarkBit || lab[j] == k));
                if (i < n && lane == 0) {
                    mlo[i] = (uint32_t)M;
                    mhi[i] = (uint32_t)(M >> 32);
// ... 163 lines not shown
                    if (x != R) {
                        nlo[t] = (uint32_t)x;
                        nhi[t] = (uint32_t)(x >> 32);
                        changed = true;
                    }
                }
                if (changed) s_over = 1u;
                __syncthreads();
                if (uni(s_over) == 0u) {
                    failed = false;
                    break;
                }
            }
            __syncthreads();
            if (failed) {
                if (threadIdx.x == 0) {
                    A.flags[k] = kFlagIncomplete;
                    atomicMin(&A.ctrl[kCtrlBarrier], k);
                    A.log_len[k] = 0u;
                }
                continue;
            }
            for (uint32_t t = threadIdx.x; t < n; t += kThreads) {
                mlo[t] = nlo[t];
                mhi[t] = nhi[t];
            }
            if (threadIdx.x == 0) atomicAdd(&A.ctrl[kCtrlLogGiveUp], 1u);
        }
        __syncthreads();
        uint32_t my_cnt = 0u;
        for (uint32_t t = threadIdx.x; t < n; t += kThreads) {
            const uint64_t V = ((uint64_t)mhi[t] << 32) | mlo[t];
            if (V != 0ull) {
                const uint32_t pos = atomicAdd(&s_nout, 1u);
                rec[3u * pos] = tid[t];
                rec[3u * pos + 1u] = (uint32_t)V;
                rec[3u * pos + 2u] = (uint32_t)(V >> 32);
            }
            my_cnt += (uint32_t)__popcll(V);
        }
        if (my_cnt) atomicAdd(&s_cnt, my_cnt);
        __syncthreads();
        RW_TICK(6)
        bool foreign = false;
        for (uint32_t i0 = (uint32_t)wave * kRwBatch; i0 < n; i0 += (uint32_t)kWaves * kRwBatch) {
            uint32_t old[kRwBatch];
#pragma unroll
            for (int j = 0; j < (int)kRwBatch; ++j) {
                old[j] = kLabelFree;
                const uint32_t i = i0 + (uint32_t)j;
                if (i < n) {
                    const uint32_t tile = tid[i];
                    const uint64_t V = ((uint64_t)mhi[i] << 32) | mlo[i];
                    if ((V >> lane) & 1ull) {
                        const size_t q = (size_t)((tile >> 16) * 8 + lr) * A.w + ((tile & 0xFFFFu) * 8 + lc);
                        old[j] = atomicMin(&A.label[q], mine);
                        A.dirty[q >> 8] = 1;
                    }
                }
            }
#pragma unroll
            for (int j = 0; j < (int)kRwBatch; ++j) {
                if (old[j] > mine) {
                    if (old[j] != kLabelFree) A.blocked[old[j] & ~kMarkBit] = 1u;
                } else if (old[j] < mine && old[j] >= kMarkBit) {
                    foreign = true;
                }
            }
        }
        if (__ballot(foreign) && lane == 0) s_blocked = 1u;
        __syncthreads();
        RW_TICK(7)
        if (threadIdx.x == 0) {
            A.count[k] = s_cnt;
            A.log_len[k] = s_nout | kLogShrunk;
            if (s_blocked) A.blocked[k] = 1u;
            A.flags[k] |= n << 8;
            atomicAdd(&A.ctrl[kCtrlLogWalks], 1u);
        }
    }
}

__global__ __launch_bounds__(64) void flood_partial_commit_kernel(FloodArgs A, uint8_t* __restrict__ dmask_rw) {
    __shared__ uint32_t s_ring[3][kRingT];
    __shared__ uint32_t s_hash[3][kHashT];
    __shared__ uint32_t s_pend[2][kPend];
    __shared__ uint8_t s_ord[kHashT];
    const int lane = threadIdx.x & 63;
    const uint32_t args = walk_args(A);
    const uint32_t* ctrl = A.ctrl;
    uint32_t c_giant = uni(ctrl[kCtrlGiantStep]);
    const uint32_t c_rounds = uni(ctrl[kCtrlRounds]), n_act = uni(ctrl[kCtrlNAct]), window = uni(ctrl[kCtrlWindow]),
                   barrier = uni(ctrl[kCtrlBarrier]);
    const uint32_t grid = gridDim.x;
    LR_PIN7(c_giant, c_rounds, n_act, window, barrier, args, grid);
    if (c_giant != 0u) return;
    const uint32_t* __restrict__ act = (c_rounds & 1u) ? A.act_b : A.act_a;
    LaneWords W = lane_words(lane);
    LdsStore L{s_ring[0], s_ring[1], s_ring[2], s_hash[0], s_hash[1], s_hash[2], s_ord};
    Pending P{s_pend[0], s_pend[1]};
    for (uint32_t ai = uni(blockIdx.x); ai < n_act; ai += grid) {
        const uint32_t k = uni(act[ai]);
        if (k >= window || k >= barrier) continue;
        uint32_t fl = uni(A.flags[k]);
        const uint32_t cnt = uni(A.count[k]), blocked = uni(A.blocked[k]), s_u = uni(A.seed_rec[k].x);
        LR_PIN4(fl, cnt, blocked, s_u);
        if ((cnt == 0u) | (blocked == 0u) | ((fl & (kFlagIncomplete | kFlagSelfFail)) != 0u)) continue;
        const int s = (int)s_u;
        const uint32_t seed_label = uni(A.label[s]);
        if (seed_label != (kMarkBit | k) && seed_label != k) continue;
        for (int i = lane; i < LdsStore::kHashN; i += 64) L.hk[i] = 0u;
        P.pt[lane] = 0u;
        const int sr = s / A.w, sc = s - sr * A.w;
        L.put(0u, ((uint32_t)(sr >> 3) << 16) | (uint32_t)(sc >> 3), 1ull << ((sr & 7) * 8 + (sc & 7)));
        WalkState st{0u, 1u, 0u, 0u, false, 0u, 0u};
        asm volatile("" : "+v"(W.c.z));
        const LaneConsts K = lane_consts(W);
        (void)walk<LdsStore, 1>(A, k, 0, 0.f, 0.f, 0.f, L, P, st, lane, K, false, dmask_rw);
    }
}

__device__ __forceinline__ bool seed_commits(const FloodArgs& A, uint32_t k, uint32_t barrier) {
    const uint32_t fl = A.flags[k];
    return A.count[k] > 0u && A.blocked[k] == 0u && !(fl & (kFlagIncomplete | kFlagSelfFail)) && k < barrier;
}

__global__ __launch_bounds__(256) void flood_commit_pixels_kernel(FloodArgs A, uint32_t* __restrict__ label, size_t npix,
                                                                  uint8_t* __restrict__ dmask) {
    const uint32_t* __restrict__ ctrl = A.ctrl;
    if (ctrl[kCtrlNAct] == 0u || ctrl[kCtrlGiantStep] != 0u) return;
    const uint32_t barrier = ctrl[kCtrlBarrier];
    const int lane = threadIdx.x & 63;
    const uint32_t n_runs = (uint32_t)((npix + 255) >> 8);
    for (uint32_t run = blockIdx.x * 4u + (threadIdx.x >> 6); run < n_runs; run += gridDim.x * 4u) {
        if (uni((uint32_t)A.dirty[run]) == 0u) continue;
        if (lane == 0) A.dirty[run] = 0;
        const size_t i0 = ((size_t)run << 8) + (size_t)lane * 4;
        uint32_t v[4] = {kLabelFree, kLabelFree, kLabelFree, kLabelFree};
        if (i0 + 3 < npix) {
            const uint4 q = *reinterpret_cast<const uint4*>(label + i0);
            v[0] = q.x, v[1] = q.y, v[2] = q.z, v[3] = q.w;
        } else {
            for (int j = 0; j < 4; ++j)
                if (i0 + j < npix) v[j] = label[i0 + j];
        }
#pragma unroll
        for (int j = 0; j < 4; ++j) {
            if (v[j] >= kMarkBit && v[j] != kLabelFree) {
                const uint32_t k = v[j] & ~kMarkBit;
                const bool committed = seed_commits(A, k, barrier);
                label[i0 + j] = committed ? k : kLabelFree;
                if (committed) dmask[i0 + j] = 0;
            }
        }
    }
}

__device__ __forceinline__ void flood_report(uint32_t* host_progress, uint32_t rounds, uint32_t n_left, bool stalled, bool want_giant,
                                             uint32_t giants_done, bool huge, bool calm = false) {
    const unsigned long long w = (unsigned long long)(n_left & 0x1FFFFFFFu) | ((unsigned long long)(stalled ? 1u : 0u) << 29) |
                                 ((unsigned long long)(want_giant ? 1u : 0u) << 30) | ((unsigned long long)(huge ? 1u : 0u) << 31) |
                                 ((unsigned long long)min(rounds, 0xFFFu) << 32) | ((unsigned long long)min(giants_done, 0xFFFFu) << 44) |
                                 ((unsigned long long)(calm ? 1u : 0u) << 60) | (1ull << 63);
    __hip_atomic_store(reinterpret_cast<unsigned long long*>(host_progress), w, __ATOMIC_RELEASE, __HIP_MEMORY_SCOPE_SYSTEM);
}

__device__ void flood_advance(uint32_t* __restrict__ ctrl, uint32_t win_shift, uint32_t* host_progress, uint32_t giant_step,
                              uint32_t giant_many) {
    const uint32_t n_act = ld_agent(&ctrl[kCtrlNAct]);
    if (n_act == 0u) {
        if (host_progress)
            flood_report(host_progress, max(ld_agent(&ctrl[kCtrlRounds]), 1u), 0u, false, false, ld_agent(&ctrl[kCtrlGiantDone]),
                         ld_agent(&ctrl[kCtrlMaxFlood]) != 0u);
        return;
    }
    const uint32_t n_seeds = ld_agent(&ctrl[kCtrlNSeeds]), win_hold = ld_agent(&ctrl[kCtrlWinHold]);
    const uint32_t n_next = ld_agent(&ctrl[kCtrlNNext]);
    const uint32_t window = ld_agent(&ctrl[kCtrlWindow]);
    const bool moved = ld_agent(&ctrl[kCtrlNCommit]) > 0u || n_next < n_act;
    const bool want_giant = giant_step != 0u && n_next > 0u && ld_agent(&ctrl[kCtrlGiantLowNext]) != 0xFFFFFFFFu &&
                            ld_agent(&ctrl[kCtrlGiantLowNext]) == ld_agent(&ctrl[kCtrlLowestNext]);
    const bool progress = moved || window < n_seeds || want_giant;
    bool staged = ld_agent(&ctrl[kCtrlStaged]) != 0u;
    unsigned long long grown = (unsigned long long)window << (staged ? 1u : win_shift);
    if (grown > n_seeds) grown = n_seeds;
    const uint32_t phase = ld_agent(&ctrl[kCtrlPhase]);
    if (n_next > 0u && giants_many(ctrl, giant_many)) {
        ctrl[kCtrlStaged] = 1u;
        ctrl[kCtrlPhase] = 2u;
        grown = n_seeds >> 2;
    } else if (phase == 0u && window >= n_seeds && win_hold < n_seeds && ld_agent(&ctrl[kCtrlBigTotal]) >= kHoldMinBig && n_next > 0u) {
        grown = win_hold;
        ctrl[kCtrlPhase] = 1u;
    } else if (phase == 1u) {
        if (window < win_hold) {
            if (grown > win_hold) grown = win_hold;
        } else {
            grown = window;
            if (ld_agent(&ctrl[kCtrlBelow]) <= kHoldRelease || !moved) {
                grown = n_seeds;
                ctrl[kCtrlPhase] = 2u;
            }
        }
    }
    {
        const uint32_t lowest = ld_agent(&ctrl[kCtrlLowestNext]), giant = ld_agent(&ctrl[kCtrlGiantLowNext]);
        const bool skip_rule = ld_agent(&ctrl[kCtrlGiantRuled]) != 0u && !moved && !want_giant;
        bool ruled = false;
        const unsigned long long grown_free = grown;
        if (giant != 0xFFFFFFFFu && !skip_rule) {
            const uint32_t n_marked = max(ld_agent(&ctrl[kCtrlGiantCountNext]), 1u);
            const unsigned long long rest = n_seeds > giant ? (unsigned long long)(n_seeds - giant) : 1ull;
            const unsigned long long line = (unsigned long long)giant + 1ull + (unsigned long long)kGiantProbes * rest / n_marked;
            (void)lowest;
            if (line < grown) {
                grown = line;
                ruled = true;
            }
        }
        const uint32_t defer = ld_agent(&ctrl[kCtrlDeferLowNext]);
        ctrl[kCtrlDeferLow] = defer;
        ctrl[kCtrlDeferLowNext] = 0xFFFFFFFFu;
        if (defer < grown && defer > lowest) grown = defer;
        ctrl[kCtrlWindowFree] = (uint32_t)grown_free;
        ctrl[kCtrlGiantRuled] = ruled ? 1u : 0u;
        ctrl[kCtrlLowest] = lowest;
        ctrl[kCtrlGiantLow] = giant;
        ctrl[kCtrlLowestNext] = 0xFFFFFFFFu;
        ctrl[kCtrlGiantLowNext] = 0xFFFFFFFFu;
        ctrl[kCtrlGiantCountNext] = 0u;
    }
    ctrl[kCtrlWindow] = (uint32_t)grown;
    ctrl[kCtrlBelow] = 0u;
    ctrl[kCtrlRounds] = ld_agent(&ctrl[kCtrlRounds]) + 1u;
    ctrl[kCtrlNRemain] = n_next;
    if (!progress) ctrl[kCtrlStall] = 1u;
    ctrl[kCtrlNAct] = progress ? n_next : 0u;
    ctrl[kCtrlNNext] = 0u;
    ctrl[kCtrlNCommit] = 0u;
    ctrl[kCtrlBarrier] = ld_agent(&ctrl[kCtrlBarrierNext]);
    ctrl[kCtrlBarrierNext] = 0xFFFFFFFFu;
    ctrl[kCtrlSlabs] = 0u;
    ctrl[kCtrlNBig] = 0u;
    ctrl[kCtrlNRewalk] = 0u;
    ctrl[kCtrlBigSeen] = ld_agent(&ctrl[kCtrlBigLong]) >= kRegionalMin ? 1u : 0u;
    ctrl[kCtrlGiantStep] = (progress && want_giant) ? ld_agent(&ctrl[kCtrlLowest]) + 1u : 0u;
    ctrl[kCtrlGiantReuse] = 0u;
    if (host_progress)
        flood_report(host_progress, ld_agent(&ctrl[kCtrlRounds]), progress ? n_next : 0u, !progress, progress && want_giant,
                     ld_agent(&ctrl[kCtrlGiantDone]), ld_agent(&ctrl[kCtrlMaxFlood]) != 0u,
                     window >= n_seeds && ld_agent(&ctrl[kCtrlBigTotal]) == 0u && ld_agent(&ctrl[kCtrlSlabTotal]) == 0u &&
                         ld_agent(&ctrl[kCtrlQuietMiss]) == 0u);
}

__global__ __launch_bounds__(256) void flood_survivors_kernel(FloodArgs A, uint8_t* __restrict__ state,
                                                              int32_t* __restrict__ seed_size) {
    if (giant_pending(A)) return;
    const uint32_t* __restrict__ act = act_now(A);
    uint32_t* __restrict__ act_next = act_other(A);
    const uint32_t n_act = A.ctrl[kCtrlNAct];
    const uint32_t n_pad = (n_act + 255u) & ~255u;
    const uint32_t window = A.ctrl[kCtrlWindow];
    const uint32_t barrier = A.ctrl[kCtrlBarrier];
    __shared__ uint32_t s_cnt[4][5];
    __shared__ uint32_t s_base;
    const int wave = threadIdx.x >> 6, lane = threadIdx.x & 63;
    for (uint32_t ai = blockIdx.x * 256 + threadIdx.x; ai < n_pad; ai += gridDim.x * 256) {
        bool a = false, done = false;
        uint32_t k = 0, wpx = 0, wst = 0, dfr = 0xFFFFFFFFu;
        if (ai < n_act) {
            k = act[ai];
            wpx = A.count[k];
            wst = A.flags[k] >> 8;
            if (A.flags[k] & kFlagSelfFail) {
                state[k] = 2;
                seed_size[k] = 0;
            } else if (seed_commits(A, k, barrier)) {
                state[k] = 2;
                seed_size[k] = (int32_t)A.count[k];
                done = true;
                if (A.count[k] > kHugeFlood) atomicMax(&A.ctrl[kCtrlMaxFlood], A.count[k]);
            } else if (state[k] == 0) {
                const uint32_t own_label = A.label[A.seed_idx[k]];
                if (own_label < kMarkBit && own_label != k) {
                    state[k] = 2;
                    seed_size[k] = 0;
                } else {
                    a = true;
                    A.blocked[k] = 0u;
                    A.count[k] = 0u;
                    A.flags[k] = 0u;
                    A.tier[k] = (uint8_t)(A.tier[k] & 5u);
                    if (A.blk != nullptr) {
                        const uint32_t bk = A.blk[k];
                        if (bk != 0xFFFFFFFFu) {
                            if (state[bk] != 0) A.blk[k] = 0xFFFFFFFFu;
                            else dfr = k;
                        }
                    }
                }
            }
        }
        const uint64_t m = __ballot(a), md = __ballot(done), mb = __ballot(a && k < window);
#pragma unroll
        for (int off = 32; off >= 1; off >>= 1) {
            wpx += (uint32_t)__shfl_xor((int)wpx, off);
            wst += (uint32_t)__shfl_xor((int)wst, off);
        }
        uint32_t kmin = a ? k : 0xFFFFFFFFu, gmin = (a && (A.tier[k] & 4u)) ? k : 0xFFFFFFFFu;
#pragma unroll
        for (int off = 32; off >= 1; off >>= 1) {
            kmin = min(kmin, (uint32_t)__shfl_xor((int)kmin, off));
            gmin = min(gmin, (uint32_t)__shfl_xor((int)gmin, off));
        }
        const uint64_t mg = __ballot(a && (A.tier[k] & 4u));
        if (__ballot(dfr != 0xFFFFFFFFu) != 0ull) {
#pragma unroll
            for (int off = 32; off >= 1; off >>= 1) dfr = min(dfr, (uint32_t)__shfl_xor((int)dfr, off));
            if (lane == 0) atomicMin(&A.ctrl[kCtrlDeferLowNext], dfr);
        }
        if (lane == 0) {
            if (kmin != 0xFFFFFFFFu) atomicMin(&A.ctrl[kCtrlLowestNext], kmin);
            if (gmin != 0xFFFFFFFFu) {
                atomicMin(&A.ctrl[kCtrlGiantLowNext], gmin);
                atomicAdd(&A.ctrl[kCtrlGiantCountNext], (uint32_t)__popcll(mg));
            }
        }
        if (lane == 0) {
            s_cnt[wave][0] = (uint32_t)__popcll(m);
            s_cnt[wave][1] = (uint32_t)__popcll(md);
            s_cnt[wave][2] = (uint32_t)__popcll(mb);
            s_cnt[wave][3] = wpx;
            s_cnt[wave][4] = wst;
        }
        __syncthreads();
        if (threadIdx.x == 0) {
            const uint32_t na = s_cnt[0][0] + s_cnt[1][0] + s_cnt[2][0] + s_cnt[3][0];
            const uint32_t nd = s_cnt[0][1] + s_cnt[1][1] + s_cnt[2][1] + s_cnt[3][1];
            const uint32_t nb = s_cnt[0][2] + s_cnt[1][2] + s_cnt[2][2] + s_cnt[3][2];
            s_base = na ? atomicAdd(&A.ctrl[kCtrlNNext], na) : 0u;
            if (nd) atomicAdd(&A.ctrl[kCtrlNCommit], nd);
            if (nb) atomicAdd(&A.ctrl[kCtrlBelow], nb);
            const uint32_t np_ = s_cnt[0][3] + s_cnt[1][3] + s_cnt[2][3] + s_cnt[3][3];
            const uint32_t ns_ = s_cnt[0][4] + s_cnt[1][4] + s_cnt[2][4] + s_cnt[3][4];
            if (np_) atomicAdd(reinterpret_cast<unsigned long long*>(&A.ctrl[kCtrlWalked]), (unsigned long long)np_);
            if (ns_) atomicAdd(reinterpret_cast<unsigned long long*>(&A.ctrl[kCtrlSteps]), (unsigned long long)ns_);
        }
        __syncthreads();
        if (a) {
            uint32_t base = s_base;
            for (int w2 = 0; w2 < wave; ++w2) base += s_cnt[w2][0];
            const uint32_t pos = base + (uint32_t)__popcll(m & ((1ull << lane) - 1ull));
            act_next[pos] = k;
            if (pos >= A.next_reach) atomicMin(&A.ctrl[kCtrlBarrierNext], k);
        }
        __syncthreads();
    }
    __shared__ uint32_t s_closed;
    __syncthreads();
    if (threadIdx.x == 0) {
        s_closed = 0u;
        __threadfence();
        if (atomicAdd(&A.ctrl[kCtrlDone], 1u) == gridDim.x - 1u) {
            __threadfence();
            A.ctrl[kCtrlDone] = 0u;
            flood_advance(A.ctrl, A.win_shift, A.host_progress, A.giant_step, A.giant_many);
            __threadfence();
            s_closed = 1u;
        }
    }
    if (A.host_ctrl == nullptr) return;
    __syncthreads();
    if (s_closed != 0u && threadIdx.x < kCtrlWords && ld_agent(&A.ctrl[kCtrlNAct]) == 0u)
        __hip_atomic_store(&A.host_ctrl[threadIdx.x], ld_agent(&A.ctrl[threadIdx.x]), __ATOMIC_RELAXED, __HIP_MEMORY_SCOPE_SYSTEM);
}

__global__ __launch_bounds__(256) void flood_init_seeds_kernel(const uint32_t* __restrict__ n_ptr, uint32_t cap,
                                                               uint32_t* __restrict__ act, uint8_t* __restrict__ state,
                                                               uint8_t* __restrict__ tier, uint32_t* __restrict__ blocked,
                                                               uint32_t* __restrict__ count, uint32_t* __restrict__ flags,
                                                               int32_t* __restrict__ seed_size, uint32_t* __restrict__ ctrl,
                                                               uint8_t* __restrict__ dirty, uint32_t n_runs,
                                                               int win_first_shift, int hold_pct, uint32_t hold_from_start,
                                                               uint32_t* __restrict__ label, size_t npix,
                                                               uint32_t* __restrict__ log_len, uint32_t log_seeds,
                                                               uint32_t staged_from_start, uint32_t* __restrict__ blk) {
    for (size_t i = (size_t)blockIdx.x * 256 + threadIdx.x; i < npix; i += (size_t)gridDim.x * 256) label[i] = kLabelFree;
    const uint32_t k = blockIdx.x * 256 + threadIdx.x;
    const uint32_t n_seeds = min(*n_ptr, cap);
    if (k == 0u) {
        uint32_t win_first = win_first_shift > 0 ? max(1024u, n_seeds >> win_first_shift) : n_seeds;
        if (win_first_shift <= 0 && n_seeds > (uint32_t)(npix / kDenseDiv)) win_first = max(1024u, n_seeds >> 3);
        if (win_first > n_seeds) win_first = n_seeds;
        uint32_t win_hold = (hold_pct > 0 && hold_pct < 100) ? (uint32_t)((unsigned long long)n_seeds * (uint32_t)hold_pct / 100u) : n_seeds;
        if (win_hold < 1024u) win_hold = n_seeds;
        const bool hold_now = hold_from_start != 0u && win_hold < n_seeds;
        if (hold_now && win_first > win_hold) win_first = win_hold;
        ctrl[kCtrlNSeeds] = n_seeds;
        ctrl[kCtrlWinHold] = win_hold;
        ctrl[kCtrlWindow] = win_first;
        ctrl[kCtrlDone] = 0u;
        ctrl[kCtrlBelow] = 0u;
        ctrl[kCtrlNBig] = 0u;
        ctrl[kCtrlBigTotal] = 0u;
        ctrl[kCtrlBigLong] = 0u;
        ctrl[kCtrlBigSeen] = 0u;
        ctrl[kCtrlNRewalk] = 0u;
        ctrl[kCtrlLowest] = 0u;
        ctrl[kCtrlLowestNext] = 0xFFFFFFFFu;
        ctrl[kCtrlGiantLow] = 0xFFFFFFFFu;
        ctrl[kCtrlGiantLowNext] = 0xFFFFFFFFu;
        ctrl[kCtrlGiantRuled] = 0u;
        ctrl[kCtrlGiantCountNext] = 0u;
        ctrl[kCtrlGiants] = 0u;
        ctrl[kCtrlGiantStep] = 0u;
        ctrl[kCtrlGiantReuse] = 0u;
        ctrl[kCtrlDeferLow] = 0xFFFFFFFFu;
        ctrl[kCtrlDeferLowNext] = 0xFFFFFFFFu;
        ctrl[kCtrlStaged] = staged_from_start;
        ctrl[kCtrlMaxFlood] = 0u;
        ctrl[kCtrlGiantDone] = 0u;
        ctrl[kCtrlGiantPx] = 0u;
        ctrl[kCtrlGiantBlocks] = 0u;
        ctrl[kCtrlLogTotal] = 0u;
        ctrl[kCtrlLogWalks] = 0u;
        ctrl[kCtrlLogGiveUp] = 0u;
        ctrl[kCtrlSlabTotal] = 0u;
        ctrl[kCtrlQuietMiss] = 0u;
        ctrl[kCtrlTeamDone] = 0u;
        ctrl[kCtrlTeamGiants] = 0u;
        ctrl[kCtrlBarrier] = 0xFFFFFFFFu;
        ctrl[kCtrlBarrierNext] = 0xFFFFFFFFu;
        ctrl[kCtrlSlabs] = 0u;
        ctrl[kCtrlNAct] = n_seeds;
        ctrl[kCtrlNCommit] = 0u;
        ctrl[kCtrlNNext] = 0u;
        ctrl[kCtrlPhase] = hold_now ? 1u : 0u;
        ctrl[kCtrlRounds] = 0u;
        ctrl[kCtrlStall] = 0u;
        ctrl[kCtrlNRemain] = n_seeds;
        ctrl[kCtrlWalked] = ctrl[kCtrlWalked + 1] = 0u;
        ctrl[kCtrlSteps] = ctrl[kCtrlSteps + 1] = 0u;
    }
    for (uint32_t r = k; r < n_runs; r += gridDim.x * 256) dirty[r] = 0;
    if (k >= n_seeds) return;
    if (k < log_seeds) log_len[k] = 0u;
    act[k] = k;
    state[k] = 0;
    tier[k] = 0;
    if (blk) blk[k] = 0xFFFFFFFFu;
    blocked[k] = 0u;
    count[k] = 0u;
    flags[k] = 0u;
    seed_size[k] = 0;
}

__device__ __forceinline__ uint64_t giant_closure(uint64_t c, uint64_t M) {
    uint64_t prev;
    do {
        prev = c;
        c = dilate8(c) & M;
        c = dilate8(c) & M;
    } while (c != prev);
    return c;
}
__device__ __forceinline__ uint32_t gu_find(uint32_t* par, uint32_t x) {
    for (;;) {
        const uint32_t p = ld_agent(&par[x]);
        if (p == x) return x;
// ... 876 lines not shown
```

### librectify_amd/csrc/kernels_groups.hip

```cpp
#include "common.h"

namespace lramd {
namespace {

constexpr int kWG = 1024;
constexpr int kWaves = kWG / 64;

__device__ __forceinline__ float wave_tree(float v) {
#pragma unroll
    for (int off = 32; off >= 1; off >>= 1) v = v + __shfl_xor(v, off);
    return v;
}

__device__ __forceinline__ uint32_t block_rank(bool flag, uint32_t* s_cnt, uint32_t& total) {
    const int lane = threadIdx.x & 63, wv = threadIdx.x >> 6;
    const uint64_t m = __ballot(flag);
    __syncthreads();
    if (lane == 0) s_cnt[wv] = (uint32_t)__popcll(m);
    __syncthreads();
    uint32_t before = 0, tot = 0;
#pragma unroll
    for (int i = 0; i < kWaves; ++i) {
        const uint32_t c = s_cnt[i];
        before += i < wv ? c : 0u;
        tot += c;
    }
    total = tot;
    return before + (uint32_t)__popcll(m & ((1ull << lane) - 1ull));
}

__device__ __forceinline__ void pencil_model_of(const LineSegment& l, uint32_t i, float cx, float cy, float sc, const PencilTable& all,
                                                const PencilTable& round0) {
    const float x1 = (l.x1 - cx) / sc, y1 = (l.y1 - cy) / sc, x2 = (l.x2 - cx) / sc, y2 = (l.y2 - cy) / sc;
    float hx = y1 * 1.f - 1.f * y2, hy = 1.f * x2 - x1 * 1.f, hz = x1 * y2 - y1 * x2;
    const float zz = (hx * hx + hy * hy) + hz * hz;
    if (zz > 0.0f) {
        const float nn = sqrtf(zz);
        hx = hx / nn;
        hy = hy / nn;
        hz = hz / nn;
    }
    const float ax = (x2 + x1) / 2, ay = (y2 + y1) / 2;
    const float dx = x2 - x1, dy = y2 - y1;
    const float len = sqrtf(dx * dx + dy * dy);
    const float ux = dx / len, uy = dy / len;
    all.ax[i] = ax; all.ay[i] = ay; all.dx[i] = ux; all.dy[i] = uy; all.len[i] = len;
    all.hx[i] = hx; all.hy[i] = hy; all.hz[i] = hz; all.orig[i] = i;
    round0.ax[i] = ax; round0.ay[i] = ay; round0.dx[i] = ux; round0.dy[i] = uy; round0.len[i] = len;
    round0.hx[i] = hx; round0.hy[i] = hy; round0.hz[i] = hz; round0.orig[i] = i;
}

__global__ __launch_bounds__(kWG) void filter_lines_kernel(const LineSegment* __restrict__ raw,
                                                           const uint32_t* __restrict__ n_raw_ptr, uint32_t raw_cap,
                                                           float min_length, LineSegment* __restrict__ out,
                                                           uint32_t* __restrict__ gctl, float* __restrict__ gnorm,
                                                           PencilTable all, PencilTable round0, uint32_t with_model) {
    constexpr int kFlB = 8;
    __shared__ uint32_t s_cnt[kFlB][kWaves];
    __shared__ float s_red[4][kWaves];
    const uint32_t n_raw = min(*n_raw_ptr, raw_cap);
    const float ml = fmaxf(min_length, kLineMinLength);
    const int lane = threadIdx.x & 63, wv = threadIdx.x >> 6;
    uint32_t base = 0;
    if (n_raw >= 2u) {
        for (uint32_t i0 = 0; i0 < n_raw; i0 += kWG * kFlB) {
            LineSegment l[kFlB];
            uint64_t m[kFlB];
#pragma unroll
            for (int b = 0; b < kFlB; ++b) {
                const uint32_t i = i0 + (uint32_t)b * kWG + threadIdx.x;
                l[b] = LineSegment{};
                if (i < n_raw) l[b] = raw[i];
            }
#pragma unroll
            for (int b = 0; b < kFlB; ++b) {
                const uint32_t i = i0 + (uint32_t)b * kWG + threadIdx.x;
                const float dx = l[b].x2 - l[b].x1, dy = l[b].y2 - l[b].y1;
                const bool keep = i < n_raw && sqrtf(dx * dx + dy * dy) > ml && l[b].err < kLineMaxErr;
                m[b] = __ballot(keep);
                if (lane == 0) s_cnt[b][wv] = (uint32_t)__popcll(m[b]);
            }
            __syncthreads();
#pragma unroll
            for (int b = 0; b < kFlB; ++b) {
                uint32_t before = 0, tot = 0;
#pragma unroll
                for (int w = 0; w < kWaves; ++w) {
                    const uint32_t c = s_cnt[b][w];
                    before += w < wv ? c : 0u;
                    tot += c;
                }
                if ((m[b] >> lane) & 1ull) {
                    l[b].group_id = -1;
                    out[base + before + (uint32_t)__popcll(m[b] & ((1ull << lane) - 1ull))] = l[b];
                }
                base += tot;
            }
            __syncthreads();
        }
    }
    __syncthreads();
    const uint32_t n = base;
    float mnx = INFINITY, mny = INFINITY, mxx = -INFINITY, mxy = -INFINITY;
    for (uint32_t i = threadIdx.x; i < n; i += kWG) {
        const LineSegment l = out[i];
        mnx = fminf(mnx, fminf(l.x1, l.x2));
        mny = fminf(mny, fminf(l.y1, l.y2));
        mxx = fmaxf(mxx, fmaxf(l.x1, l.x2));
        mxy = fmaxf(mxy, fmaxf(l.y1, l.y2));
    }
#pragma unroll
    for (int off = 32; off >= 1; off >>= 1) {
        mnx = fminf(mnx, __shfl_xor(mnx, off));
        mny = fminf(mny, __shfl_xor(mny, off));
        mxx = fmaxf(mxx, __shfl_xor(mxx, off));
        mxy = fmaxf(mxy, __shfl_xor(mxy, off));
    }
    if ((threadIdx.x & 63) == 0) {
        s_red[0][threadIdx.x >> 6] = mnx;
        s_red[1][threadIdx.x >> 6] = mny;
        s_red[2][threadIdx.x >> 6] = mxx;
        s_red[3][threadIdx.x >> 6] = mxy;
    }
    __syncthreads();
    if (threadIdx.x == 0) {
        for (int i = 1; i < kWaves; ++i) {
            mnx = fminf(mnx, s_red[0][i]);
            mny = fminf(mny, s_red[1][i]);
            mxx = fmaxf(mxx, s_red[2][i]);
            mxy = fmaxf(mxy, s_red[3][i]);
        }
        const float sx = mxx - mnx, sy = mxy - mny;
        gnorm[0] = mnx + 0.5f * sx;
        gnorm[1] = mny + 0.5f * sy;
        gnorm[2] = fmaxf(sx, sy);
        gctl[kGcLines] = n;
        gctl[kGcRemaining] = n;
        gctl[kGcRound] = 0u;
        gctl[kGcActive] = n;
// ... 223 lines not shown
            const float hv[3] = {hl.x, hl.y, hl.z};
#pragma unroll
            for (int a = 0; a < 3; ++a) {
                const float t = hv[a] * hl.w;
#pragma unroll
                for (int b = 0; b < 3; ++b) acc[a * 3 + b] = acc[a * 3 + b] + t * hv[b];
            }
        }
#pragma unroll
        for (int k = 0; k < 9; ++k) acc[k] = wave_tree(acc[k]);
#ifdef LR_PEEL_TIMING
        tm[3] = wall_clock64();
#endif
        if (lane == 0) {
            float hf[3];
            smallest_eigenvector_3x3(acc, hf);
            s_h[0] = hf[0];
            s_h[1] = hf[1];
            s_h[2] = hf[2];
            if (round < (uint32_t)kMaxPeelModels) {
                models[round * 3 + 0] = hf[0];
                models[round * 3 + 1] = hf[1];
                models[round * 3 + 2] = hf[2];
            }
        }
    }
    __syncthreads();
    const float fx = s_h[0], fy = s_h[1], fz = s_h[2];
#ifdef LR_PEEL_TIMING
    tm[4] = wall_clock64();
#endif

    uint32_t n_next = 0, n_gone = 0;
    for (uint32_t i0 = 0; i0 < n; i0 += kWG) {
        const uint32_t i = i0 + threadIdx.x;
        bool stay = false, gone = false;
        if (i < n) {
            if (i0 != 0) {
                r_ax = cur.ax[i]; r_ay = cur.ay[i]; r_dx = cur.dx[i]; r_dy = cur.dy[i]; r_len = cur.len[i];
                r_hx = cur.hx[i]; r_hy = cur.hy[i]; r_hz = cur.hz[i]; r_orig = cur.orig[i];
            }
            const float e = pencil_error(r_ax, r_ay, r_dx, r_dy, fx, fy, fz);
            if (e < tol) {
                lines[r_orig].group_id = (int)round;
                gone = true;
            } else if (e >= tol && e < garbage_tol) {
                gone = true;
            } else {
                stay = true;
            }
        }
        uint32_t tot, tg;
        const uint32_t r = block_rank(stay, s_cnt, tot);
        if (stay) {
            const uint32_t o = n_next + r;
            nxt.ax[o] = r_ax; nxt.ay[o] = r_ay; nxt.dx[o] = r_dx; nxt.dy[o] = r_dy;
            nxt.len[o] = r_len; nxt.hx[o] = r_hx; nxt.hy[o] = r_hy; nxt.hz[o] = r_hz;
            nxt.orig[o] = r_orig;
        }
        (void)block_rank(gone, s_cnt, tg);
        n_next += tot;
        n_gone += tg;
    }
#ifdef LR_PEEL_TIMING
    if (threadIdx.x == 0) {
        tm[5] = wall_clock64();
        for (int q = 0; q < 5 && round < 4u; ++q) models[16 + round * 5 + q] = (float)(tm[q + 1] - tm[q]) * 0.01f;
    }
#endif
    if (threadIdx.x == 0) {
        gctl[kGcActive] = n_next;
        gctl[kGcRemaining] = gctl[kGcRemaining] - n_gone;
        gctl[kGcRound] = round + 1u;
    }
}

__global__ __launch_bounds__(kWG) void peel_kernel(PencilTable cur, PencilTable nxt, PencilTable all,
                                                   unsigned long long* __restrict__ best_slots, uint64_t seed,
                                                   float tol, float garbage_tol, int max_models,
                                                   uint32_t* __restrict__ gctl, float4* __restrict__ stage_g,
                                                   LineSegment* __restrict__ lines, float* __restrict__ models,
                                                   const uint32_t* __restrict__ counts, uint32_t cap_lines,
                                                   uint32_t* __restrict__ gather_dst) {
    peel_body(cur, nxt, all, best_slots, seed, tol, garbage_tol, max_models, gctl, stage_g, lines, models);
    if (gather_dst == nullptr) return;
    __syncthreads();
    const uint32_t t = threadIdx.x;
    const uint32_t* gw = gctl;
    if (t < 8) gather_dst[t] = counts[t];
    else if (t < 16) gather_dst[t] = gw[t - 8];
    else if (t < 56) gather_dst[t] = reinterpret_cast<const uint32_t*>(models)[t - 16];
    const uint32_t n = min(gw[kGcLines], cap_lines) * (uint32_t)(sizeof(LineSegment) / 4);
    const uint32_t* lw = reinterpret_cast<const uint32_t*>(lines);
    for (uint32_t i = t; i < n; i += kWG) gather_dst[64 + i] = lw[i];
}

}

int launch_filter_lines(const LineSegment* raw, const uint32_t* d_n_raw, uint32_t raw_cap, float min_length,
                        LineSegment* out, uint32_t* gctl, float* gnorm, const PencilTable* all, const PencilTable* round0,
                        hipStream_t s) {
    const bool with_model = all != nullptr && round0 != nullptr;
    hipLaunchKernelGGL(filter_lines_kernel, dim3(1), dim3(kWG), 0, s, raw, d_n_raw, raw_cap, min_length, out, gctl, gnorm,
                       with_model ? *all : PencilTable{}, with_model ? *round0 : PencilTable{}, with_model ? 1u : 0u);
    LR_HIP(hipGetLastError());
    return 0;
}

int launch_lines_bbox(LineSegment* lines, uint32_t n, uint32_t* gctl, float* gnorm, hipStream_t s) {
    hipLaunchKernelGGL(lines_bbox_kernel, dim3(1), dim3(kWG), 0, s, lines, n, gctl, gnorm);
    LR_HIP(hipGetLastError());
    return 0;
}

int launch_pencil_model(const LineSegment* lines, const uint32_t* gctl, const float* gnorm, PencilTable all,
                        PencilTable round0, uint32_t line_cap, hipStream_t s) {
    if (line_cap == 0) return 0;
    hipLaunchKernelGGL(pencil_model_kernel, dim3((line_cap + 255) / 256), dim3(256), 0, s, lines, gctl, gnorm, all, round0);
    LR_HIP(hipGetLastError());
    return 0;
}

int launch_peel(PencilTable cur, PencilTable nxt, PencilTable all, unsigned long long* best_slots, uint64_t seed,
                float tol, float garbage_tol, int max_models, uint32_t* gctl, float* stage4, LineSegment* lines,
                float* models, const uint32_t* counts, uint32_t cap_lines, void* gather_block, hipStream_t s) {
    hipLaunchKernelGGL(peel_kernel, dim3(1), dim3(kWG), 0, s, cur, nxt, all, best_slots, seed, tol, garbage_tol,
                       max_models, gctl, reinterpret_cast<float4*>(stage4), lines, models, counts, cap_lines,
                       static_cast<uint32_t*>(gather_block));
    LR_HIP(hipGetLastError());
    return 0;
}

}
```

### librectify_amd/csrc/kernels_ransac.hip

```cpp
#include <cstdlib>

#include "common.h"

namespace lramd {
namespace {

__device__ inline float wave_tree(float v) {
#pragma unroll
    for (int off = 32; off >= 1; off >>= 1) v = v + __shfl_xor(v, off);
    return v;
}

constexpr float kErrBand = 3e-6f;

__device__ __forceinline__ bool inlier_exact(float vx, float vy, float dx, float dy, float tol) {
    const float nn = vx * vx + vy * vy;
    const float nrm = sqrtf(nn);
    const float ux = vx / nrm, uy = vy / nrm;
    const float inc = fabsf(ux * dx + uy * dy);
    const float err = -inc + 1.0f;
    return err < tol;
}

__device__ __forceinline__ bool inlier_test(float vx, float vy, float dx, float dy, float tol) {
    const float nn = __builtin_fmaf(vx, vx, vy * vy);
    const float dot = __builtin_fmaf(vx, dx, vy * dy);
    const float e = 1.0f - fabsf(dot) * __builtin_amdgcn_rsqf(nn);
    bool in = e < tol - kErrBand;
    const bool sure = (in || e > tol + kErrBand) && nn > 1e-30f;
    if (__builtin_expect(!sure, 0)) in = inlier_exact(vx, vy, dx, dy, tol);
    return in;
}

struct Hyp {
    float cx, cy, sub;
    bool valid;
};
__device__ __forceinline__ Hyp make_hyp(const PencilSoA& m, uint32_t a, uint32_t b, float degeneracy_tol) {
    const float hax = m.hx[a], hay = m.hy[a], haz = m.hz[a];
    const float hbx = m.hx[b], hby = m.hy[b], hbz = m.hz[b];
    const float ex = hax - hbx, ey = hay - hby, ez = haz - hbz;
    const float dist = sqrtf((ex * ex + ey * ey) + ez * ez);
    Hyp h;
    h.valid = dist > degeneracy_tol;
    const float px = hay * hbz - haz * hby;
    const float py = haz * hbx - hax * hbz;
    const float pz = hax * hby - hay * hbx;
    const bool ideal = fabsf(pz) < kEps;
    h.cx = ideal ? px : px / pz;
    h.cy = ideal ? py : py / pz;
    h.sub = ideal ? 0.f : 1.f;
    return h;
}
__device__ __forceinline__ void hyp_v(const Hyp& h, float ax, float ay, float& vx, float& vy) {
    vx = h.sub != 0.f ? h.cx - ax : h.cx;
    vy = h.sub != 0.f ? h.cy - ay : h.cy;
}

constexpr float kTiny = 1e-30f;
struct EstConst {
    float k_in, k_out;
};
__device__ __forceinline__ EstConst est_const(float tol) {
    const float a = (1.0f - tol) + kErrBand, b = (1.0f - tol) - kErrBand;
    return EstConst{a * a, b * b};
}
typedef float f2 __attribute__((ext_vector_type(2)));
__device__ __forceinline__ void inlier_estimate2(const f2 cx, const f2 cy, const f2 nsub, float ax, float ay, float dx, float dy,
                                                 const EstConst& K, uint64_t& m_in0, uint64_t& m_un0, uint64_t& m_in1,
                                                 uint64_t& m_un1) {
    const f2 vx = __builtin_elementwise_fma(nsub, (f2){ax, ax}, cx), vy = __builtin_elementwise_fma(nsub, (f2){ay, ay}, cy);
    const f2 nn = __builtin_elementwise_fma(vx, vx, vy * vy);
    const f2 dot = __builtin_elementwise_fma(vx, (f2){dx, dx}, vy * (f2){dy, dy});
    const f2 dd = dot * dot;
    const f2 t_in = __builtin_elementwise_fma(nn, (f2){K.k_in, K.k_in}, (f2){kTiny, kTiny});
    const f2 t_out = __builtin_elementwise_fma(nn, (f2){K.k_out, K.k_out}, (f2){-kTiny, -kTiny});
    m_in0 = __builtin_amdgcn_fcmpf(dd.x, t_in.x, 2);
    m_in1 = __builtin_amdgcn_fcmpf(dd.y, t_in.y, 2);
    m_un0 = ~(m_in0 | __builtin_amdgcn_fcmpf(dd.x, t_out.x, 4));
    m_un1 = ~(m_in1 | __builtin_amdgcn_fcmpf(dd.y, t_out.y, 4));
}

constexpr int kScoreChunk = 512;
constexpr uint32_t kBestSlots = (uint32_t)kRansacBestSlots;
template <int kH>
__global__ __launch_bounds__(256) void ransac_score_kernel(PencilSoA m, uint32_t n_host, float tol, float degeneracy_tol,
                                                           uint32_t n_iter, uint64_t seed, uint32_t round_host,
                                                           const uint32_t* __restrict__ gctl, int max_models,
                                                           unsigned long long* __restrict__ best_slots) {
    __shared__ float s_tab[2][5][kScoreChunk];
    __shared__ unsigned long long s_key[4];
    const int lane = threadIdx.x & 63;
    const uint32_t hyp0 = (blockIdx.x * 4 + (threadIdx.x >> 6)) * kH;
    if (blockIdx.x * 4u * kH >= n_iter) return;
    uint32_t n = n_host, round = round_host;
    if (gctl) {
        n = gctl[kGcActive];
        round = gctl[kGcRound];
        if (gctl[kGcRemaining] < 2u || round >= (uint32_t)max_models) return;
    }
    float cx[kH], cy[kH], nsub[kH];
    bool valid[kH];
#pragma unroll
    for (int j = 0; j < kH; ++j) {
        uint32_t a, b;
        sample_pair(seed, round, min(hyp0 + (uint32_t)j, n_iter - 1u), n, a, b);
        const Hyp h = make_hyp(m, a, b, degeneracy_tol);
        cx[j] = h.cx;
        cy[j] = h.cy;
        nsub[j] = -h.sub;
        valid[j] = h.valid;
    }
    const EstConst K = est_const(tol);
    float acc[kH];
#pragma unroll
    for (int j = 0; j < kH; ++j) acc[j] = 0.f;
    auto stage = [&](int buf, uint32_t c0) {
        for (uint32_t t = threadIdx.x; t < (uint32_t)kScoreChunk; t += 256) {
            const uint32_t i = c0 + t;
            if (i < n) {
                s_tab[buf][0][t] = m.ax[i];
                s_tab[buf][1][t] = m.ay[i];
                s_tab[buf][2][t] = m.dx[i];
                s_tab[buf][3][t] = m.dy[i];
                s_tab[buf][4][t] = m.len[i];
            }
        }
    };
    stage(0, 0u);
    int buf = 0;
    for (uint32_t c0 = 0; c0 < n; c0 += kScoreChunk, buf ^= 1) {
        __syncthreads();
        if (c0 + kScoreChunk < n) stage(buf ^ 1, c0 + kScoreChunk);
        const uint32_t cn = min((uint32_t)kScoreChunk, n - c0);
        for (uint32_t t = lane; t < cn; t += 64) {
            const float ax = s_tab[buf][0][t], ay = s_tab[buf][1][t], dx = s_tab[buf][2][t], dy = s_tab[buf][3][t];
            const float len = s_tab[buf][4][t];
            uint64_t any_unsure = 0ull, mu[kH];
            static_assert(kH % 2 == 0, "hypotheses are scored in pairs");
#pragma unroll
            for (int j = 0; j < kH; j += 2) {
                uint64_t mi0, mi1;
                inlier_estimate2((f2){cx[j], cx[j + 1]}, (f2){cy[j], cy[j + 1]}, (f2){nsub[j], nsub[j + 1]}, ax, ay, dx, dy, K, mi0,
                                 mu[j], mi1, mu[j + 1]);
                acc[j] = acc[j] + (__builtin_amdgcn_inverse_ballot_w64(mi0 & ~mu[j]) ? len : 0.0f);
                acc[j + 1] = acc[j + 1] + (__builtin_amdgcn_inverse_ballot_w64(mi1 & ~mu[j + 1]) ? len : 0.0f);
                any_unsure |= mu[j] | mu[j + 1];
            }
            if (__builtin_expect(any_unsure != 0ull, 0)) {
#pragma unroll
                for (int j = 0; j < kH; ++j)
                    if (__builtin_amdgcn_inverse_ballot_w64(mu[j])) {
                        const float vx = __builtin_fmaf(nsub[j], ax, cx[j]), vy = __builtin_fmaf(nsub[j], ay, cy[j]);
                        acc[j] = acc[j] + (inlier_exact(vx, vy, dx, dy, tol) ? len : 0.0f);
                    }
            }
        }
    }
    unsigned long long key = 0ull;
#pragma unroll
    for (int j = 0; j < kH; ++j) {
        const float score = wave_tree(acc[j]);
        const uint32_t it = hyp0 + (uint32_t)j;
        if (valid[j] && it < n_iter && score > 0.0f) {
            const unsigned long long k = ((unsigned long long)__float_as_uint(score) << 32) | (unsigned long long)(0xFFFFFFFFu - it);
            key = k > key ? k : key;
        }
    }
    if (lane == 0) s_key[threadIdx.x >> 6] = key;
    __syncthreads();
    if (threadIdx.x != 0) return;
    for (int wv = 1; wv < 4; ++wv) key = s_key[wv] > key ? s_key[wv] : key;
// ... 539 lines not shown
```

### librectify_amd/csrc/kernels_seeds.hip

```cpp
#include <algorithm>
#include <cstdlib>
#include <cstring>

#include "common.h"

namespace lramd {
namespace {

__global__ __launch_bounds__(256) void seed_count_kernel(const uint64_t* __restrict__ cand,
                                                         const uint32_t* __restrict__ cand_count,
                                                         const uint32_t* __restrict__ tile_max, int n_tiles, int cand_cap,
                                                         float keep_ratio, float* __restrict__ maxmag,
                                                         uint32_t* __restrict__ tile_pass) {
    __shared__ uint32_t s_red[4];
    const int lane = threadIdx.x & 63, wave = threadIdx.x >> 6;
    uint32_t m = 0;
    for (int i0 = threadIdx.x; i0 < n_tiles; i0 += 256 * 8) {
        uint32_t v[8];
#pragma unroll
        for (int k = 0; k < 8; ++k) {
            const int i = i0 + k * 256;
            v[k] = i < n_tiles ? tile_max[i] : 0u;
        }
#pragma unroll
// ... 17 lines not shown
    if (lane == 0) tile_pass[tile] = cnt;
}

__global__ __launch_bounds__(1024) void seed_scan_kernel(const uint32_t* __restrict__ tile_pass, int n_tiles,
                                                         uint32_t* __restrict__ tile_off, uint32_t* __restrict__ n_seeds) {
    __shared__ uint32_t s_wave[16];
    const int lane = threadIdx.x & 63, wave = threadIdx.x >> 6;
    const int K = (n_tiles + 1023) / 1024;
    const int i0 = (int)threadIdx.x * K, i1 = min(n_tiles, i0 + K);
    uint32_t sum = 0;
    for (int b0 = i0; b0 < i1; b0 += 8) {
        uint32_t v[8];
#pragma unroll
        for (int k = 0; k < 8; ++k) v[k] = b0 + k < i1 ? tile_pass[b0 + k] : 0u;
#pragma unroll
        for (int k = 0; k < 8; ++k) sum += v[k];
    }
    uint32_t inc = sum;
#pragma unroll
    for (int off = 1; off < 64; off <<= 1) {
        const uint32_t o = (uint32_t)__shfl_up((int)inc, off);
        if (lane >= off) inc += o;
    }
    if (lane == 63) s_wave[wave] = inc;
    __syncthreads();
    uint32_t before = 0, total = 0;
#pragma unroll
    for (int w2 = 0; w2 < 16; ++w2) {
        const uint32_t t = s_wave[w2];
        before += w2 < wave ? t : 0u;
        total += t;
    }
    uint32_t run = before + inc - sum;
    for (int b0 = i0; b0 < i1; b0 += 8) {
        uint32_t v[8];
#pragma unroll
        for (int k = 0; k < 8; ++k) v[k] = b0 + k < i1 ? tile_pass[b0 + k] : 0u;
#pragma unroll
        for (int k = 0; k < 8; ++k)
            if (b0 + k < i1) {
                tile_off[b0 + k] = run;
                run += v[k];
            }
    }
    if (threadIdx.x == 0) *n_seeds = total;
}

__global__ __launch_bounds__(256) void seed_write_kernel(const uint64_t* __restrict__ cand,
                                                         const uint32_t* __restrict__ cand_count, int n_tiles,
                                                         int cand_cap, const float* __restrict__ maxmag,
                                                         float keep_ratio, const uint32_t* __restrict__ tile_pass,
                                                         const uint32_t* __restrict__ tile_off,
                                                         uint64_t* __restrict__ keys, uint32_t cap) {
    const int tile = blockIdx.x * 4 + (threadIdx.x >> 6);
    const int lane = threadIdx.x & 63;
    if (tile >= n_tiles) return;
    const float thr = *maxmag * keep_ratio;
    const uint32_t n = cand_count[tile];
    const uint64_t* c = cand + (size_t)tile * cand_cap;
    uint32_t base = tile_off[tile];
    for (uint32_t i0 = 0; i0 < n; i0 += 64) {
        const uint32_t i = i0 + lane;
        uint64_t k = 0;
        bool pass = false;
        if (i < n) {
            k = c[i];
            pass = __uint_as_float((uint32_t)(k >> 32)) > thr;
        }
        const uint64_t m = __ballot(pass);
        if (pass) {
            const uint32_t pos = base + (uint32_t)__popcll(m & ((1ull << lane) - 1ull));
            if (pos < cap) keys[pos] = ((uint64_t)(~(uint32_t)(k >> 32)) << 32) | (k & 0xFFFFFFFFull);
        }
        base += (uint32_t)__popcll(m);
    }
}

constexpr int kSelBands = 2048;
__global__ __launch_bounds__(256) void seed_select_kernel(const uint64_t* __restrict__ cand, const uint32_t* __restrict__ cand_count,
                                                          const uint32_t* __restrict__ tile_max, int n_tiles, int cand_cap, int per_wg,
                                                          float keep_ratio, float* __restrict__ maxmag,
                                                          unsigned long long* __restrict__ status, uint32_t tag,
                                                          uint64_t* __restrict__ keys, uint32_t cap, uint32_t* __restrict__ n_seeds) {
    __shared__ uint32_t s_red[4], s_sum[4];
    __shared__ uint32_t s_cnt[kSelBands];
    __shared__ uint32_t s_total;
    const int lane = threadIdx.x & 63, wave = threadIdx.x >> 6;
    uint32_t m = 0;
    for (int i0 = threadIdx.x; i0 < n_tiles; i0 += 256 * 8) {
        uint32_t v[8];
#pragma unroll
        for (int k = 0; k < 8; ++k) {
            const int i = i0 + k * 256;
            v[k] = i < n_tiles ? tile_max[i] : 0u;
        }
#pragma unroll
        for (int k = 0; k < 8; ++k) m = max(m, v[k]);
    }
#pragma unroll
    for (int off = 32; off >= 1; off >>= 1) m = max(m, (uint32_t)__shfl_xor((int)m, off));
    if (lane == 0) s_red[wave] = m;
    __syncthreads();
    const float mx = __uint_as_float(max(max(s_red[0], s_red[1]), max(s_red[2], s_red[3])));
    if (blockIdx.x == 0 && threadIdx.x == 0) *maxmag = mx;
    const float thr = mx * keep_ratio;
    const int t0 = (int)blockIdx.x * per_wg, t1 = min(n_tiles, t0 + per_wg);
    for (int t = t0 + wave; t < t1; t += 4) {
        const uint32_t n = cand_count[t];
        const uint64_t* c = cand + (size_t)t * cand_cap;
        uint32_t cnt = 0;
        for (uint32_t i = lane; i < n; i += 64) cnt += (__uint_as_float((uint32_t)(c[i] >> 32)) > thr) ? 1u : 0u;
#pragma unroll
        for (int off = 32; off >= 1; off >>= 1) cnt += (uint32_t)__shfl_xor((int)cnt, off);
        if (lane == 0) s_cnt[t - t0] = cnt;
    }
    __syncthreads();
    const int nb = max(t1 - t0, 0);
    if (wave == 0) {
        uint32_t run = 0;
        for (int c0 = 0; c0 < nb; c0 += 64) {
            const uint32_t v = c0 + lane < nb ? s_cnt[c0 + lane] : 0u;
            uint32_t inc = v;
#pragma unroll
            for (int off = 1; off < 64; off <<= 1) {
                const uint32_t o = (uint32_t)__shfl_up((int)inc, off);
                if (lane >= off) inc += o;
            }
            if (c0 + lane < nb) s_cnt[c0 + lane] = run + inc - v;
            run += (uint32_t)__shfl((int)inc, 63);
        }
        if (lane == 0) {
            s_total = run;
            __hip_atomic_store(&status[blockIdx.x], ((unsigned long long)tag << 32) | (unsigned long long)run, __ATOMIC_RELAXED,
                               __HIP_MEMORY_SCOPE_AGENT);
        }
    }
    uint32_t before = 0;
    for (uint32_t j = threadIdx.x; j < blockIdx.x; j += 256) {
        unsigned long long w = 0ull;
        for (uint32_t spins = 0; spins < (1u << 22); ++spins) {
            w = __hip_atomic_load(&status[j], __ATOMIC_RELAXED, __HIP_MEMORY_SCOPE_AGENT);
            if ((uint32_t)(w >> 32) == tag) break;
            __builtin_amdgcn_s_sleep(2);
        }
        before += (uint32_t)w;
    }
#pragma unroll
    for (int off = 32; off >= 1; off >>= 1) before += (uint32_t)__shfl_xor((int)before, off);
    if (lane == 0) s_sum[wave] = before;
    __syncthreads();
    const uint32_t base0 = s_sum[0] + s_sum[1] + s_sum[2] + s_sum[3];
    if (blockIdx.x == gridDim.x - 1 && threadIdx.x == 0) *n_seeds = base0 + s_total;
    for (int t = t0 + wave; t < t1; t += 4) {
        const uint32_t n = cand_count[t];
        const uint64_t* c = cand + (size_t)t * cand_cap;
        uint32_t base = base0 + s_cnt[t - t0];
        for (uint32_t i0 = 0; i0 < n; i0 += 64) {
            const uint32_t i = i0 + lane;
            uint64_t k = 0;
            bool pass = false;
            if (i < n) {
                k = c[i];
                pass = __uint_as_float((uint32_t)(k >> 32)) > thr;
            }
            const uint64_t mm = __ballot(pass);
            if (pass) {
                const uint32_t pos = base + (uint32_t)__popcll(mm & ((1ull << lane) - 1ull));
                if (pos < cap) keys[pos] = ((uint64_t)(~(uint32_t)(k >> 32)) << 32) | (k & 0xFFFFFFFFull);
            }
            base += (uint32_t)__popcll(mm);
        }
    }
}

constexpr uint32_t kRun0 = 2048;
constexpr uint32_t kRunThreads = kRun0 / 4;
constexpr uint32_t kFinalRuns = 16;

__device__ __forceinline__ uint64_t shfl_xor_u64(uint64_t v, int lane_mask) {
    const uint32_t lo = (uint32_t)__shfl_xor((int)(uint32_t)v, lane_mask);
    const uint32_t hi = (uint32_t)__shfl_xor((int)(uint32_t)(v >> 32), lane_mask);
    return ((uint64_t)hi << 32) | lo;
}
__global__ __launch_bounds__(kRunThreads) void seed_run_sort_kernel(uint64_t* __restrict__ keys, uint32_t cap,
                                                            const uint32_t* __restrict__ n_ptr) {
    __shared__ uint64_t sk[kRun0];
    const uint32_t n = min(*n_ptr, cap);
    const uint32_t base = blockIdx.x * kRun0;
    if (base >= n) return;
    const uint32_t t = threadIdx.x, i0 = 4u * t;
    uint64_t e[4];
#pragma unroll
    for (int r = 0; r < 4; ++r) e[r] = (base + i0 + r < n) ? keys[base + i0 + r] : ~0ull;
#define LR_KEEP(own, other, i, j, k) ((((((i) & (j)) == 0u) == (((i) & (k)) == 0u)) == ((other) < (own))) ? (other) : (own))
    for (uint32_t k = 2; k <= kRun0; k <<= 1) {
        for (uint32_t j = k >> 1; j > 0; j >>= 1) {
            if (j >= 256u) {
#pragma unroll
                for (int r = 0; r < 4; ++r) sk[i0 + r] = e[r];
                __syncthreads();
                uint64_t o[4];
#pragma unroll
                for (int r = 0; r < 4; ++r) o[r] = sk[(i0 + r) ^ j];
                __syncthreads();
#pragma unroll
                for (int r = 0; r < 4; ++r) e[r] = LR_KEEP(e[r], o[r], i0 + r, j, k);
            } else if (j >= 4u) {
                const int lm = (int)(j >> 2);
#pragma unroll
                for (int r = 0; r < 4; ++r) {
                    const uint64_t o = shfl_xor_u64(e[r], lm);
                    e[r] = LR_KEEP(e[r], o, i0 + r, j, k);
                }
            } else {
                const bool two = j == 2u;
                const uint64_t o0 = two ? e[2] : e[1], o1 = two ? e[3] : e[0], o2 = two ? e[0] : e[3], o3 = two ? e[1] : e[2];
                e[0] = LR_KEEP(e[0], o0, i0 + 0u, j, k);
                e[1] = LR_KEEP(e[1], o1, i0 + 1u, j, k);
                e[2] = LR_KEEP(e[2], o2, i0 + 2u, j, k);
                e[3] = LR_KEEP(e[3], o3, i0 + 3u, j, k);
            }
        }
    }
#undef LR_KEEP
#pragma unroll
    for (int r = 0; r < 4; ++r)
        if (base + i0 + r < n) keys[base + i0 + r] = e[r];
}

__device__ __forceinline__ uint32_t count_below(const uint64_t* __restrict__ run, uint32_t L, uint32_t valid, uint64_t key) {
    uint32_t lo = 0;
    for (uint32_t sstep = L >> 1; sstep > 0; sstep >>= 1) {
        const uint32_t pos = lo + sstep - 1u;
        const uint64_t v = pos < valid ? run[pos] : ~0ull;
        lo += v < key ? sstep : 0u;
    }
    return lo + ((lo == L - 1u && L - 1u < valid && run[L - 1u] < key) ? 1u : 0u);
}

__global__ __launch_bounds__(256) void seed_merge_kernel(const uint64_t* __restrict__ in, uint64_t* __restrict__ out, uint32_t L,
                                                         uint32_t cap, const uint32_t* __restrict__ n_ptr) {
    const uint32_t g = blockIdx.x * 256 + threadIdx.x;
    const uint32_t n = min(*n_ptr, cap);
    if (g >= n) return;
    const uint32_t r = g / L, i = g - r * L, q = r ^ 1u;
    const uint64_t key = in[g];
    const uint32_t qbase = q * L;
    const uint32_t valid = qbase < n ? min(L, n - qbase) : 0u;
    const uint32_t below = valid ? count_below(in + qbase, L, valid, key) : 0u;
    out[(size_t)(r & ~1u) * L + i + below] = key;
}

__global__ __launch_bounds__(256) void seed_rank_setup_kernel(const uint64_t* __restrict__ keys, const uint32_t* __restrict__ n_ptr,
                                                              uint32_t cap, uint32_t L, const float* __restrict__ dx,
                                                              const float* __restrict__ dy, BinTrig trig, float trace_tolerance,
                                                              int32_t* __restrict__ seed_idx, int32_t* __restrict__ seed_bin,
                                                              float* __restrict__ seed_thr, uint4* __restrict__ seed_rec) {
    const uint32_t g = blockIdx.x * 256 + threadIdx.x;
    const uint32_t n = min(*n_ptr, cap);
    if (g >= n) return;
    const uint32_t n_runs = (n + L - 1u) / L;
    const uint32_t mine = g / L;
    const uint64_t key = keys[g];
    uint32_t rank = g - mine * L;
    for (uint32_t q0 = 0; q0 < n_runs; q0 += 8u) {
        uint32_t lo[8], valid[8];
#pragma unroll
        for (int j = 0; j < 8; ++j) {
            const uint32_t q = q0 + (uint32_t)j;
            lo[j] = 0u;
            valid[j] = (q < n_runs && q != mine) ? min(L, n - q * L) : 0u;
        }
        for (uint32_t sstep = L >> 1; sstep > 0; sstep >>= 1) {
            uint64_t v[8];
#pragma unroll
            for (int j = 0; j < 8; ++j) {
                const uint32_t pos = lo[j] + sstep - 1u;
                v[j] = pos < valid[j] ? keys[(size_t)(q0 + (uint32_t)j) * L + pos] : ~0ull;
            }
#pragma unroll
            for (int j = 0; j < 8; ++j) lo[j] += v[j] < key ? sstep : 0u;
        }
#pragma unroll
        for (int j = 0; j < 8; ++j) {
            if (lo[j] == L - 1u && L - 1u < valid[j] && keys[(size_t)(q0 + (uint32_t)j) * L + L - 1u] < key) lo[j] += 1u;
            rank += lo[j];
        }
    }
    const uint32_t low = (uint32_t)key;
    const uint32_t idx = low >> 3;
    const int bin = (int)(low & 7u);
    const float v = directional(dx[idx], dy[idx], trig.st[bin], trig.ct[bin]);
    seed_idx[rank] = (int32_t)idx;
    seed_bin[rank] = bin;
    const float thr = (1 - trace_tolerance) * v;
    seed_thr[rank] = thr;
    seed_rec[rank] = make_uint4(idx, (uint32_t)bin, __float_as_uint(thr), 0u);
}

}

int launch_seed_order(uint64_t* keys, uint64_t* keys_alt, const uint32_t* n_seeds, uint32_t cap, const float* dx, const float* dy,
                      BinTrig trig, float trace_tolerance, int32_t* seed_idx, int32_t* seed_bin, float* seed_thr, uint4* seed_rec, hipStream_t s) {
    if (cap == 0) return 0;
    const uint32_t runs0 = (cap + kRun0 - 1) / kRun0;
    hipLaunchKernelGGL(seed_run_sort_kernel, dim3(runs0), dim3(kRunThreads), 0, s, keys, cap, n_seeds);
    uint32_t L = kRun0, runs = runs0;
    uint64_t* cur = keys;
    uint64_t* nxt = keys_alt;
    while (runs > 1u && (runs > kFinalRuns || (uint64_t)cap * runs > ((uint64_t)4 << 20))) {
        hipLaunchKernelGGL(seed_merge_kernel, dim3((cap + 255) / 256), dim3(256), 0, s, cur, nxt, L, cap, n_seeds);
        std::swap(cur, nxt);
        L *= 2u;
        runs = (runs + 1u) / 2u;
    }
    hipLaunchKernelGGL(seed_rank_setup_kernel, dim3((cap + 255) / 256), dim3(256), 0, s, cur, n_seeds, cap, L, dx, dy, trig,
                       trace_tolerance, seed_idx, seed_bin, seed_thr, seed_rec);
    LR_HIP(hipGetLastError());
    return 0;
}

size_t seeds_temp_bytes(int n_tiles, size_t max_seeds) {
    (void)n_tiles;
    (void)max_seeds;
    return 256;
}

int launch_seed_select(const uint64_t* cand, const uint32_t* cand_count, const uint32_t* tile_max, int n_tiles,
                       int cand_cap, float seed_keep_ratio, float* maxmag, uint32_t* tile_pass, uint32_t* tile_off, uint64_t* keys,
                       uint32_t key_cap, uint32_t* n_seeds, uint32_t frame_tag, hipStream_t s) {
    static const bool fused = !(std::getenv("LIBRECTIFY_SEED_SELECT_FUSED") && std::atoi(std::getenv("LIBRECTIFY_SEED_SELECT_FUSED")) == 0);
    if (fused && frame_tag != 0u && n_tiles > 0) {
        int wgs = std::min(256, (n_tiles + 3) / 4);
        int per_wg = (n_tiles + wgs - 1) / wgs;
        if (per_wg > kSelBands) {
            per_wg = kSelBands;
            wgs = (n_tiles + per_wg - 1) / per_wg;
        }
        wgs = (n_tiles + per_wg - 1) / per_wg;
        hipLaunchKernelGGL(seed_select_kernel, dim3(wgs), dim3(256), 0, s, cand, cand_count, tile_max, n_tiles, cand_cap, per_wg,
// ... 16 lines not shown
```

Measured before the change: 10570.

## Defer per-frame rectification transform until next frame's kernels are enqueued

Each lane now writes its line results right away but holds the vanishing-point/rectification transform for a frame until the lane's next frame has been enqueued on the GPU. A hook fires after enqueue, so the host-side transform math overlaps GPU execution instead of sitting between frames. The diff also adds wave-priority hints (s_setprio) to many kernels, dropped during spin-waits, but these compile only when LR_CHAIN_PRIO_ON is defined. The deferral adds a std::function hook per context and keeps a copy of one frame's results per lane.

```diff
diff --git a/librectify_amd/csrc/batch.hip b/librectify_amd/csrc/batch.hip
--- a/librectify_amd/csrc/batch.hip
+++ b/librectify_amd/csrc/batch.hip
@@ -41,6 +41,7 @@
         for (lr_context* l : lanes) {
             l->sleep_in_wait = false;
             l->keep_workspace = false;
+            l->enqueued_hook = nullptr;
         }
         c->flood_logbig_off = false;
         c->flood_log_min = c->flood_log_walk = 0;
@@ -60,25 +61,48 @@
     int* n_lines;
     const RectificationConfig* cfg;
     ImageTransform* transforms;
-    void write(int b, const std::vector<LineSegment>& res, int w, int h) const {
+    void write_lines(int b, const std::vector<LineSegment>& res) const {
         const int n = (int)res.size();
         if (n_lines) n_lines[b] = n;
         if (out && capacity > 0 && n > 0) std::memcpy(out + (size_t)b * capacity, res.data(), sizeof(LineSegment) * (size_t)std::min(n, capacity));
-        if (transforms) {
-            const RectificationConfig def;
-            transforms[b] = rectification_transform(res.data(), std::min(n, capacity > 0 ? capacity : n), w, h, cfg ? *cfg : def);
-        }
+    }
+    void write_transform(int b, const std::vector<LineSegment>& res, int w, int h) const {
+        if (!transforms) return;
+        const int n = (int)res.size();
+        const RectificationConfig def;
+        transforms[b] = rectification_transform(res.data(), std::min(n, capacity > 0 ? capacity : n), w, h, cfg ? *cfg : def);
     }
 };
 
+struct LaneOut {
+    const BatchOut& to;
+    int b = -1, w = 0, h = 0;
+    std::vector<LineSegment> res;
+    explicit LaneOut(const BatchOut& o) : to(o) {}
+    void finish(int b_, std::vector<LineSegment>& r, int w_, int h_) {
+        flush();
+        to.write_lines(b_, r);
+        if (!to.transforms) return;
+        res.swap(r);
+        b = b_, w = w_, h = h_;
+    }
+    void flush() {
+        if (b < 0) return;
+        to.write_transform(b, res, w, h);
+        b = -1;
+    }
+};
+
 template <class Frame>
-static int run_lanes(const LaneSet& lanes, int batch, std::atomic<int>& stop, const Frame& frame) {
+static int run_lanes(const LaneSet& lanes, int batch, std::atomic<int>& stop, const BatchOut& results, const Frame& frame) {
     const int S = lanes.size();
     std::atomic<int> next_frame{0};
     std::vector<int> rc((size_t)S, 0);
     std::vector<std::string> err((size_t)S);
     auto work = [&](int si) {
         bool failed = false;
+        LaneOut lane_out(results);
+        lanes[si]->enqueued_hook = [&lane_out]() { lane_out.flush(); };
         if (si > 0 && hipSetDevice(lanes[0]->device) != hipSuccess) {
             set_error("hipSetDevice failed");
             failed = true;
@@ -86,8 +110,10 @@
         while (!failed && !stop.load(std::memory_order_relaxed)) {
             const int b = next_frame.fetch_add(1, std::memory_order_relaxed);
             if (b >= batch) break;
-            failed = frame(lanes[si], si, b) != 0;
-        }
+            failed = frame(lanes[si], si, b, lane_out) != 0;
+        }
+        lanes[si]->enqueued_hook = nullptr;
+        lane_out.flush();
         if (failed) {
             rc[(size_t)si] = 1;
             err[(size_t)si] = get_error();
@@ -120,12 +146,12 @@
     if (lanes.setup(c, std::max(1, std::min(c->opt.batch_streams, batch)), false, false)) return 1;
     const BatchOut results{out, capacity, n_lines, cfg, transforms};
     std::atomic<int> stop{0};
-    return run_lanes(lanes, batch, stop, [&](lr_context* l, int, int b) {
+    return run_lanes(lanes, batch, stop, results, [&](lr_context* l, int, int b, LaneOut& lane_out) {
         std::vector<LineSegment> res;
         if (ctx_find_groups_device(l, static_cast<const uint8_t*>(d_images) + (size_t)b * image_stride * bpp, format, w, h, stride, min_length,
                                    refine, res))
             return 1;
-        results.write(b, res, w, h);
+        lane_out.finish(b, res, w, h);
         return 0;
     });
 }
@@ -167,13 +193,13 @@
         if (ctx_reserve_workspace(lanes[si], max_pix, max_tiles)) return 1;
     const BatchOut results{out, capacity, n_lines, cfg, transforms};
     std::atomic<int> stop{0};
-    return run_lanes(lanes, batch, stop, [&](lr_context* l, int, int b) {
+    return run_lanes(lanes, batch, stop, results, [&](lr_context* l, int, int b, LaneOut& lane_out) {
         const lr_frame& f = frames[b];
         std::vector<LineSegment> res;
         if (f.width >= 5 && f.height >= 5 &&
             ctx_find_groups_device(l, f.data, format, f.width, f.height, f.stride, f.min_length < 0.f ? min_length : f.min_length, refine, res))
             return 1;
-        results.write(b, res, f.width, f.height);
+        lane_out.finish(b, res, f.width, f.height);
         return 0;
     });
 }
@@ -193,7 +219,7 @@
     LaneSet lanes;
     if (lanes.setup(c, S, true, false) || up.start()) return 1;
     const BatchOut results{out, capacity, n_lines, cfg, transforms};
-    const int lanes_rc = run_lanes(lanes, batch, up.stop, [&](lr_context* l, int si, int b) {
+    const int lanes_rc = run_lanes(lanes, batch, up.stop, results, [&](lr_context* l, int si, int b, LaneOut& lane_out) {
         const void* img = nullptr;
         int slot = -1;
         if (up.ready(b, l->stream, &img, &slot)) return 1;
@@ -202,7 +228,7 @@
         const double t_f0 = now_ms();
         if (ctx_find_groups_device(l, img, format, w, h, w, min_length, refine, res)) return 1;
         up.release(slot, b, l, si, t_f0);
-        results.write(b, res, w, h);
+        lane_out.finish(b, res, w, h);
         return 0;
     });
     const std::string& up_err = up.end();
diff --git a/librectify_amd/csrc/common.h b/librectify_amd/csrc/common.h
--- a/librectify_amd/csrc/common.h
+++ b/librectify_amd/csrc/common.h
@@ -65,6 +65,12 @@
     a = i < j ? i : j;
     b = i < j ? j : i;
 }
+
+#if defined(__HIP_DEVICE_COMPILE__) && defined(LR_CHAIN_PRIO_ON)
+#define LR_CHAIN_PRIO(n) __builtin_amdgcn_s_setprio(n)
+#else
+#define LR_CHAIN_PRIO(n) ((void)0)
+#endif
 
 void set_error(const std::string& msg);
 
diff --git a/librectify_amd/csrc/context.h b/librectify_amd/csrc/context.h
--- a/librectify_amd/csrc/context.h
+++ b/librectify_amd/csrc/context.h
@@ -135,6 +135,7 @@
     std::unique_ptr<lramd::StagingCrew> crew;
     int crew_helpers = 0;
     bool sleep_in_wait = false;
+    std::function<void()> enqueued_hook;
     uint32_t fit_tag = 0;
     bool batch_no_register = false;
     int register_slow_calls = 0;
diff --git a/librectify_amd/csrc/frame.hip b/librectify_amd/csrc/frame.hip
--- a/librectify_amd/csrc/frame.hip
+++ b/librectify_amd/csrc/frame.hip
@@ -413,6 +413,7 @@
         if (enqueue_fit(c)) return 1;
         if (after_fit()) return 1;
         const double t_enq = now_ms();
+        if (attempt == 0 && c->enqueued_hook) c->enqueued_hook();
         const double t_pre = now_ms();
         if (c->sleep_in_wait) {
             LR_HIP(hipEventRecord(c->ev_wait, c->stream));
diff --git a/librectify_amd/csrc/kernels_filter.hip b/librectify_amd/csrc/kernels_filter.hip
--- a/librectify_amd/csrc/kernels_filter.hip
+++ b/librectify_amd/csrc/kernels_filter.hip
@@ -172,6 +172,7 @@
                                                            uint64_t* __restrict__ cand, uint32_t* __restrict__ cand_count,
                                                            uint32_t* __restrict__ tile_max, int bands_x, int band_begin,
                                                            int band_end) {
+    LR_CHAIN_PRIO(1);
     const int lane = threadIdx.x & 63;
 #ifndef LR_NO_XCD_ORDER
     const int chunk = (int)gridDim.x / 8;
diff --git a/librectify_amd/csrc/kernels_fit.hip b/librectify_amd/csrc/kernels_fit.hip
--- a/librectify_amd/csrc/kernels_fit.hip
+++ b/librectify_amd/csrc/kernels_fit.hip
@@ -41,6 +41,7 @@
                                                                 uint32_t large_cap, uint32_t* __restrict__ n_large,
                                                                 uint32_t* __restrict__ cursor, uint32_t* __restrict__ huge_list,
                                                                 uint32_t huge_max) {
+    LR_CHAIN_PRIO(2);
     __shared__ uint32_t s_c[4], s_p[4], s_cc[4], s_cp[4];
     const uint32_t n_seeds = min(*n_ptr, cap);
     const int tid = threadIdx.x, lane = tid & 63, wv = tid >> 6;
@@ -78,6 +79,7 @@
         }
     }
     uint32_t cc = 0, cp = 0;
+    LR_CHAIN_PRIO(0);
     for (uint32_t i = (uint32_t)tid; i < blockIdx.x; i += 256) {
         unsigned long long wc = 0ull, wp = 0ull;
         for (uint32_t spins = 0; spins < (1u << 22); ++spins) {
@@ -89,6 +91,7 @@
         cc += (uint32_t)wc;
         cp += (uint32_t)wp;
     }
+    LR_CHAIN_PRIO(2);
 #pragma unroll
     for (int off = 32; off >= 1; off >>= 1) {
         cc += (uint32_t)__shfl_xor((int)cc, off);
@@ -143,6 +146,7 @@
                                                                 uint32_t* __restrict__ cursor,
                                                                 uint32_t* __restrict__ px, uint32_t* __restrict__ huge_tab,
                                                                 uint32_t nb) {
+    LR_CHAIN_PRIO(1);
     const int lane = threadIdx.x & 63;
     const size_t step = (size_t)gridDim.x * 256;
     const size_t n_pad = (npix + 255) / 256 * 256;
@@ -239,6 +243,7 @@
                                                                    const uint32_t* __restrict__ comp_off,
                                                                    const uint32_t* __restrict__ large_list,
                                                                    const uint32_t* __restrict__ n_large) {
+    LR_CHAIN_PRIO(1);
     __shared__ uint32_t s_key[kSortLds];
     const uint32_t n_list = n_large[0];
     for (uint32_t li = blockIdx.x; li < n_list; li += gridDim.x) {
@@ -264,6 +269,7 @@
                                                                   const uint32_t* __restrict__ n_large,
                                                                   uint32_t* __restrict__ scratch,
                                                                   const uint32_t* __restrict__ cursor) {
+    LR_CHAIN_PRIO(1);
     __shared__ uint32_t s_key[kGlobal ? 1 : kSortLdsBig];
     const uint32_t n_list = n_large[1];
     for (uint32_t li = blockIdx.x; li < n_list; li += gridDim.x) {
@@ -495,6 +501,7 @@
                                                   const float* __restrict__ dy, int w, BinTrig trig,
                                                   float* __restrict__ scratch_w, LineSegment* __restrict__ out,
                                                   const uint32_t* __restrict__ huge_cursor) {
+    LR_CHAIN_PRIO(1);
     const int lane = threadIdx.x & 63;
     const uint32_t comp = blockIdx.x * 4 + (threadIdx.x >> 6);
     if (comp >= *n_comp_ptr) return;
diff --git a/librectify_amd/csrc/kernels_flood.hip b/librectify_amd/csrc/kernels_flood.hip
--- a/librectify_amd/csrc/kernels_flood.hip
+++ b/librectify_amd/csrc/kernels_flood.hip
@@ -1117,6 +1117,7 @@
                    c_staged = uni(ctrl[kCtrlStaged]);
     const uint32_t grid = gridDim.x;
     LR_PIN10(c_giant, c_rounds, n_act, window, c_seen, c_nbig, lowest, c_staged, args, grid);
+    if (!kRest && c_rounds != 0u) LR_CHAIN_PRIO(1);
     if (c_giant != 0u) return;
     const uint32_t* __restrict__ act = (c_rounds & 1u) ? A.act_b : A.act_a;
     const bool staged = c_staged != 0u;
@@ -1437,6 +1438,7 @@
 constexpr size_t kTeamLdsBytes = (size_t)(3 * kRingTeam + 3 * kHashBig + 2 * kPend) * 4 + (size_t)kHashBig * 2 + sizeof(TeamShared);
 __global__ __launch_bounds__(64 * kTeamWaves) void flood_explore_team_kernel(FloodArgs A, BinTrig trig,
                                                                              const uint32_t* __restrict__ big_list) {
+    LR_CHAIN_PRIO(1);
     extern __shared__ uint32_t s_team[];
     const int lane = threadIdx.x & 63, wave = (int)uni(threadIdx.x >> 6);
     const uint32_t args = walk_args(A);
@@ -1699,6 +1701,7 @@
 #endif
 template <int kThreads, int kTiles>
 __global__ __launch_bounds__(kThreads) void flood_rewalk_kernel(FloodArgs A, const uint32_t* __restrict__ list, uint32_t min_len) {
+    LR_CHAIN_PRIO(1);
     constexpr int kNodes = 2 * kTiles, kHash = 2 * kTiles, kWaves = kThreads / 64, kEdges = 4 * kTiles;
     static_assert(kNodes <= 65536, "node pairs are packed into 32 bits");
     constexpr int kHashShift = 32 - __builtin_ctz((unsigned)kHash);
@@ -2028,6 +2031,7 @@
 }
 
 __global__ __launch_bounds__(64) void flood_partial_commit_kernel(FloodArgs A, uint8_t* __restrict__ dmask_rw) {
+    LR_CHAIN_PRIO(1);
     __shared__ uint32_t s_ring[3][kRingT];
     __shared__ uint32_t s_hash[3][kHashT];
     __shared__ uint32_t s_pend[2][kPend];
@@ -2073,6 +2077,7 @@
 
 __global__ __launch_bounds__(256) void flood_commit_pixels_kernel(FloodArgs A, uint32_t* __restrict__ label, size_t npix,
                                                                   uint8_t* __restrict__ dmask) {
+    LR_CHAIN_PRIO(2);
     const uint32_t* __restrict__ ctrl = A.ctrl;
     if (ctrl[kCtrlNAct] == 0u || ctrl[kCtrlGiantStep] != 0u) return;
     const uint32_t barrier = ctrl[kCtrlBarrier];
@@ -2201,6 +2206,7 @@
 
 __global__ __launch_bounds__(256) void flood_survivors_kernel(FloodArgs A, uint8_t* __restrict__ state,
                                                               int32_t* __restrict__ seed_size) {
+    LR_CHAIN_PRIO(2);
     if (giant_pending(A)) return;
     const uint32_t* __restrict__ act = act_now(A);
     uint32_t* __restrict__ act_next = act_other(A);
@@ -2331,6 +2337,7 @@
                                                                uint32_t* __restrict__ label, size_t npix,
                                                                uint32_t* __restrict__ log_len, uint32_t log_seeds,
                                                                uint32_t staged_from_start, uint32_t* __restrict__ blk) {
+    LR_CHAIN_PRIO(2);
     for (size_t i = (size_t)blockIdx.x * 256 + threadIdx.x; i < npix; i += (size_t)gridDim.x * 256) label[i] = kLabelFree;
     const uint32_t k = blockIdx.x * 256 + threadIdx.x;
     const uint32_t n_seeds = min(*n_ptr, cap);
diff --git a/librectify_amd/csrc/kernels_groups.hip b/librectify_amd/csrc/kernels_groups.hip
--- a/librectify_amd/csrc/kernels_groups.hip
+++ b/librectify_amd/csrc/kernels_groups.hip
@@ -55,6 +55,7 @@
                                                            float min_length, LineSegment* __restrict__ out,
                                                            uint32_t* __restrict__ gctl, float* __restrict__ gnorm,
                                                            PencilTable all, PencilTable round0, uint32_t with_model) {
+    LR_CHAIN_PRIO(2);
     constexpr int kFlB = 8;
     __shared__ uint32_t s_cnt[kFlB][kWaves];
     __shared__ float s_red[4][kWaves];
@@ -444,6 +445,7 @@
                                                    LineSegment* __restrict__ lines, float* __restrict__ models,
                                                    const uint32_t* __restrict__ counts, uint32_t cap_lines,
                                                    uint32_t* __restrict__ gather_dst) {
+    LR_CHAIN_PRIO(2);
     peel_body(cur, nxt, all, best_slots, seed, tol, garbage_tol, max_models, gctl, stage_g, lines, models);
     if (gather_dst == nullptr) return;
     __syncthreads();
diff --git a/librectify_amd/csrc/kernels_ransac.hip b/librectify_amd/csrc/kernels_ransac.hip
--- a/librectify_amd/csrc/kernels_ransac.hip
+++ b/librectify_amd/csrc/kernels_ransac.hip
@@ -88,6 +88,7 @@
                                                            uint32_t n_iter, uint64_t seed, uint32_t round_host,
                                                            const uint32_t* __restrict__ gctl, int max_models,
                                                            unsigned long long* __restrict__ best_slots) {
+    LR_CHAIN_PRIO(1);
     __shared__ float s_tab[2][5][kScoreChunk];
     __shared__ unsigned long long s_key[4];
     const int lane = threadIdx.x & 63;
diff --git a/librectify_amd/csrc/kernels_seeds.hip b/librectify_amd/csrc/kernels_seeds.hip
--- a/librectify_amd/csrc/kernels_seeds.hip
+++ b/librectify_amd/csrc/kernels_seeds.hip
@@ -123,6 +123,7 @@
                                                           float keep_ratio, float* __restrict__ maxmag,
                                                           unsigned long long* __restrict__ status, uint32_t tag,
                                                           uint64_t* __restrict__ keys, uint32_t cap, uint32_t* __restrict__ n_seeds) {
+    LR_CHAIN_PRIO(2);
     __shared__ uint32_t s_red[4], s_sum[4];
     __shared__ uint32_t s_cnt[kSelBands];
     __shared__ uint32_t s_total;
@@ -177,6 +178,7 @@
         }
     }
     uint32_t before = 0;
+    LR_CHAIN_PRIO(0);
     for (uint32_t j = threadIdx.x; j < blockIdx.x; j += 256) {
         unsigned long long w = 0ull;
         for (uint32_t spins = 0; spins < (1u << 22); ++spins) {
@@ -186,6 +188,7 @@
         }
         before += (uint32_t)w;
     }
+    LR_CHAIN_PRIO(2);
 #pragma unroll
     for (int off = 32; off >= 1; off >>= 1) before += (uint32_t)__shfl_xor((int)before, off);
     if (lane == 0) s_sum[wave] = before;
@@ -225,6 +228,7 @@
 }
 __global__ __launch_bounds__(kRunThreads) void seed_run_sort_kernel(uint64_t* __restrict__ keys, uint32_t cap,
                                                             const uint32_t* __restrict__ n_ptr) {
+    LR_CHAIN_PRIO(2);
     __shared__ uint64_t sk[kRun0];
     const uint32_t n = min(*n_ptr, cap);
     const uint32_t base = blockIdx.x * kRun0;
@@ -281,6 +285,7 @@
 
 __global__ __launch_bounds__(256) void seed_merge_kernel(const uint64_t* __restrict__ in, uint64_t* __restrict__ out, uint32_t L,
                                                          uint32_t cap, const uint32_t* __restrict__ n_ptr) {
+    LR_CHAIN_PRIO(2);
     const uint32_t g = blockIdx.x * 256 + threadIdx.x;
     const uint32_t n = min(*n_ptr, cap);
     if (g >= n) return;
@@ -297,6 +302,7 @@
                                                               const float* __restrict__ dy, BinTrig trig, float trace_tolerance,
                                                               int32_t* __restrict__ seed_idx, int32_t* __restrict__ seed_bin,
                                                               float* __restrict__ seed_thr, uint4* __restrict__ seed_rec) {
+    LR_CHAIN_PRIO(2);
     const uint32_t g = blockIdx.x * 256 + threadIdx.x;
     const uint32_t n = min(*n_ptr, cap);
     if (g >= n) return;
```

Result: no change. 10550 (-0.2%).
